# victorca25/iNNfer

Measured on AMD Instinct MI355X. Metric: output MPix/s, 4x ESRGAN RRDB-23 1080p->4K, higher is better.
Workload: dtype f16; 1 GPU; ESRGAN RRDBNet-23 4x fp16, 1x3x1080x1920 -> 1x3x4320x7680, un-tiled (Model(chop=False)), one frame per rank; band_rows=0, parallelism=single GPU

## Files before the change

include/innfer_amd.h:

```cpp
#ifndef INNFER_AMD_H
#define INNFER_AMD_H

#include <stddef.h>
#include <stdint.h>

#ifdef __cplusplus
extern "C" {
#endif

typedef enum {
    INNFER_OK = 0,
    INNFER_ERR_INVALID = -1,
    INNFER_ERR_HIP = -2,
    INNFER_ERR_UNSUPPORTED = -3,
    INNFER_ERR_NOMEM = -4,
    INNFER_ERR_WORKSPACE = -5
} innfer_status;

typedef enum { INNFER_F16 = 0, INNFER_F32 = 1, INNFER_U8 = 2  } innfer_dtype;

typedef struct innfer_net* innfer_net_t;

#define INNFER_ABI_VERSION 122
int innfer_version(void);
const char* innfer_last_error(void);


int innfer_rrdbnet_create(innfer_net_t* out, int in_nc, int out_nc, int nf, int nb,
                          int gc, int scale, int plus);

int innfer_rrdbnet_create_ex(innfer_net_t* out, int in_nc, int out_nc, int nf, int nb,
                             int gc, int scale, int plus, int nr, int act, int pixelshuffle_up);

int innfer_rrdbnet_create_ex2(innfer_net_t* out, int in_nc, int out_nc, int nf, int nb,
                              int gc, int scale, int plus, int nr, int act, int pixelshuffle_up, int unshuffle);
int innfer_first_conv_unshuffle(const void* d_in, int in_dtype, int normalize, int fp16_mode, int N, int in_nc, int H, int W, int unshuffle,
                                const float* h_weight_oihw, const float* h_bias, int K, int act, void* d_slab, int64_t group_stride, int64_t lo, void* stream);

int innfer_srresnet_create(innfer_net_t* out, int in_nc, int out_nc, int nf, int nb, int scale);
int innfer_srresnet_create_ex(innfer_net_t* out, int in_nc, int out_nc, int nf, int nb, int scale, int act, float res_scale, int upconv_up);
int innfer_net_set_conv_input_map(innfer_net_t net, int idx, const float* h_alpha, const float* h_shift, int act);

int innfer_compact_create(innfer_net_t* out, int in_nc, int out_nc, int nf, int num_conv, int scale);
int innfer_net_set_conv_slope(innfer_net_t net, int idx, const float* h_slope);

int innfer_net_set_precision(innfer_net_t net, int fp32);

void innfer_net_destroy(innfer_net_t net);

int innfer_net_num_convs(innfer_net_t net);
int innfer_net_conv_info(innfer_net_t net, int idx, char* key, size_t key_cap, int* K, int* C);

int innfer_net_set_conv(innfer_net_t net, int idx, const float* h_weight_oihw, const float* h_bias);

int innfer_net_scale(innfer_net_t net);
size_t innfer_net_workspace_bytes(innfer_net_t net, int N, int H, int W);

int innfer_net_forward(innfer_net_t net, const void* d_in, int in_dtype, void* d_out, int out_dtype,
                       int N, int H, int W, void* d_workspace, size_t workspace_bytes, void* stream);

int innfer_net_forward_timed(innfer_net_t net, const void* d_in, int in_dtype, void* d_out, int out_dtype,
                             int N, int H, int W, void* d_workspace, size_t workspace_bytes, void* stream,
                             int cap, float* h_ms, double* h_flops, double* h_bytes, int* h_kind, int* n_launches);

int innfer_net_set_u8_io(innfer_net_t net, int normalize, int fp16_mode);

int innfer_net_set_band_rows(innfer_net_t net, int rows);

int innfer_net_set_residual_lds(innfer_net_t net, int on);

int innfer_net_set_fused_tail(innfer_net_t net, int on);
int innfer_net_set_hr_chain(innfer_net_t net, int on);

int innfer_net_set_upconv_phases(innfer_net_t net, int mode);

int innfer_net_set_final_act(innfer_net_t net, int act);

int innfer_net_set_outm(innfer_net_t net, int outm);

double innfer_net_flops(innfer_net_t net, int N, int H, int W);

typedef struct innfer_unet* innfer_unet_t;
int innfer_unet_create(innfer_unet_t* out, int in_nc, int out_nc, int num_downs, int ngf);
int innfer_unet_create_ex(innfer_unet_t* out, int in_nc, int out_nc, int num_downs, int ngf, int instance_norm, int upconv);
void innfer_unet_destroy(innfer_unet_t u);
int innfer_unet_num_params(innfer_unet_t u);
int innfer_unet_param_info(innfer_unet_t u, int idx, char* key, size_t key_cap, int* ndim, int* shape4);
int innfer_unet_set_param(innfer_unet_t u, int idx, const float* h_data);
int innfer_unet_set_eval(innfer_unet_t u, int eval_mode);
int innfer_unet_set_precision(innfer_unet_t u, int fp32);
size_t innfer_unet_workspace_bytes(innfer_unet_t u, int N, int H, int W);
double innfer_unet_flops(innfer_unet_t u, int N, int H, int W);
int innfer_unet_forward(innfer_unet_t u, const void* d_in, int in_dtype, void* d_out, int out_dtype,
                        int N, int H, int W, void* d_workspace, size_t workspace_bytes, void* stream);

typedef struct innfer_pan* innfer_pan_t;
int innfer_pan_create(innfer_pan_t* out, int in_nc, int out_nc, int nf, int unf, int nb, int scale);
int innfer_pan_create_ex(innfer_pan_t* out, int in_nc, int out_nc, int nf, int unf, int nb, int scale, int self_attention, int double_scpa, int bilinear_up);
void innfer_pan_destroy(innfer_pan_t p);
int innfer_pan_num_params(innfer_pan_t p);
int innfer_pan_param_info(innfer_pan_t p, int idx, char* key, size_t key_cap, int* ndim, int* shape4);
int innfer_pan_set_param(innfer_pan_t p, int idx, const float* h_data);
size_t innfer_pan_workspace_bytes(innfer_pan_t p, int N, int H, int W);
int innfer_pan_set_fused_scpa(innfer_pan_t p, int on);
int innfer_pan_set_precision(innfer_pan_t p, int fp32);
int innfer_pan_forward(innfer_pan_t p, const void* d_in, int in_dtype, void* d_out, int out_dtype,
                       int N, int H, int W, void* d_workspace, size_t workspace_bytes, void* stream);

typedef struct innfer_ppon* innfer_ppon_t;
int innfer_ppon_create(innfer_ppon_t* out, int in_nc, int out_nc, int nf, int nb, int scale, float alpha);
void innfer_ppon_destroy(innfer_ppon_t p);
int innfer_ppon_num_params(innfer_ppon_t p);
int innfer_ppon_param_info(innfer_ppon_t p, int idx, char* key, size_t key_cap, int* ndim, int* shape4);
int innfer_ppon_set_param(innfer_ppon_t p, int idx, const float* h_data);
size_t innfer_ppon_workspace_bytes(innfer_ppon_t p, int N, int H, int W);
int innfer_ppon_set_precision(innfer_ppon_t p, int fp32);
int innfer_ppon_forward(innfer_ppon_t p, const void* d_in, int in_dtype, void* d_out_c, void* d_out_s, void* d_out_p,
                        int out_dtype, int N, int H, int W, void* d_workspace, size_t workspace_bytes, void* stream);

typedef struct innfer_resnet* innfer_resnet_t;
int innfer_resnet_create(innfer_resnet_t* out, int in_nc, int out_nc, int ngf, int n_blocks);
int innfer_resnet_create_ex(innfer_resnet_t* out, int in_nc, int out_nc, int ngf, int n_blocks, int padding, int use_dropout, int upconv, int batch_norm);
// ... 32 lines not shown
    const void* d_packed; const float* d_bias;
    void* d_out; int64_t out_group_stride; int out_ch_off; int K;
    int N, H, W;
    int act; int upsample2x;
    const void* d_res1; int64_t res1_group_stride; float res1_scale;
    const void* d_res2; int64_t res2_group_stride; float res2_scale;
    int row_begin, row_end;
    int reflect_pad;
    int dilation;
    int dilation_groups;
    int pixel_shuffle2;
    int stride2_k4;
    int transposed2x;
    int column7;
    int split;
    int64_t in_lo, out_lo, res1_lo, res2_lo;
    int reserved0;
    int res1_from_input;
    int plane_rows;
    float* d_stats_part;
    int64_t stats_part_floats;
    int conv1x1;
    int prefix_lrelu;
    const void* d_gate_packed;
    const float* d_gate_bias;
    int in_relu;
    int conv7x7;
    int out_planar;
    int out_denorm, out_round16;
    int planar_phases;
    int outm;
} innfer_conv_args;

size_t innfer_conv3x3_packed_bytes(int K, int C);
int innfer_pack_conv3x3(const float* h_weight_oihw, int K, int C, void* h_packed);
int innfer_pack_conv3x3_rows(const float* h_weight_oihw, int K, int C, int plane_rows, void* h_packed);
int innfer_pack_convt2x_rows(const float* h_weight_iohw, int K, int C, int k, int plane_rows, void* h_packed);
int innfer_pack_conv3x3_shuffle2(const float* h_weight_oihw, const float* h_bias, int K, int C, void* h_packed, float* h_bias_out);
size_t innfer_conv7x1_packed_bytes(int K, int C);
int innfer_pack_conv7x1(const float* h_weight_oc7, int K, int C, void* h_packed);
size_t innfer_conv4x4s2_packed_bytes(int K, int C);
int innfer_pack_conv4x4s2(const float* h_weight_oihw, int K, int C, void* h_packed);
size_t innfer_convt2x_packed_bytes(int K, int C);
int innfer_pack_convt2x(const float* h_weight_iohw, int K, int C, int k, void* h_packed);
size_t innfer_conv1x1_packed_bytes(int K, int C);
int innfer_pack_conv1x1(const float* h_weight_oi, int K, int C, void* h_packed);
int innfer_pack_conv1x1_split(const float* h_weight_oi, int K, int C, void* h_packed);
int innfer_pack_selfgate(const float* h_weight_32x32, void* h_packed_2k);
size_t innfer_conv7x7_packed_bytes(int K, int C);
int innfer_pack_conv7x7(const float* h_weight_oihw, int K, int C, void* h_packed);
int innfer_pack_up2x_phases(const float* h_weight_oihw, int K, int C, int plane_rows, void* h_packed);
int innfer_conv3x3_f16(const innfer_conv_args* a, void* stream);
int innfer_conv3x3_f16_slope(const innfer_conv_args* a, const float* d_slope, void* stream);
int innfer_shuffle_add(const void* d_slab, int64_t group_stride, const void* d_base, int base_dtype, int normalize, void* d_out, int out_dtype,
                       int N, int C, int H, int W, int scale, void* stream);
int innfer_pack_conv3x3_split(const float* h_weight_oihw, int K, int C, void* h_packed);

typedef struct {
    const float* d_in; int64_t in_nstride, in_cstride; int C, Hin, Win;
    const float* d_packed; const float* d_bias; int K;
    float* d_out; int64_t out_nstride, out_cstride, out_pstride; int Wout;
    int Ho, Wo;
    int osy, osx, ooy, oox;
    int isy, isx;
    int ntap, dy[49], dx[49];
    int pad_mode;
    int up;
    int in_act;
    int act;
    float oscale;
    const float* d_res; int64_t res_nstride, res_cstride;
    const float* d_mul; int64_t mul_nstride, mul_cstride;
    int N;
    int phase_k;
    int form;
} innfer_f32conv_args;

size_t innfer_f32conv_packed_floats(int K, int C, int ntap);
int innfer_pack_f32conv(const float* h_w, int K, int C, int ntap, float* h_packed);
int innfer_f32conv(const innfer_f32conv_args* a, void* stream);
int innfer_f32conv_plan(const innfer_f32conv_args* a, int* plan);
int innfer_f32_norm(const float* d_in, int64_t in_ns, int64_t in_cs, float* d_out, int64_t out_ns, int64_t out_cs, int N, int C, int64_t HW, int mode, float eps,
                    const float* d_weight, const float* d_bias, const float* d_rmean, const float* d_rvar, int act,
                    const float* d_res, int64_t res_ns, int64_t res_cs, int form, void* stream);

int innfer_conv_stats_records(int H, int W, int phases);
int innfer_norm_combine_parts(const float* d_part, int nper, int64_t HW, float eps, const float* d_gamma, const float* d_beta, float* d_alpha, float* d_shift,
                              int C, int N, void* stream);
int innfer_norm_stats(const void* d_src, int slab, int64_t gs, int cpad, int64_t HW, float eps, const float* d_gamma, const float* d_beta, float* d_alpha, float* d_shift,
                      int C, int N, float* d_part, int64_t part_floats, void* stream);
int innfer_resnet_post_slab_parts(const void* d_src, int64_t gs, int C, int64_t HW, int N, const float* d_part, int nper, const float* d_gamma, const float* d_beta,
                                  int relu, const void* d_res, void* d_dst, void* stream);
int innfer_unet_post_slab_parts(const void* d_src, int64_t src_gs, int C, int64_t HW, int N, const float* d_part, int nper, const float* d_gamma, const float* d_beta,
                                void* d_dst0, int64_t dst0_gs, int dst0_coff, int act0, void* d_dst1, int64_t dst1_gs, int dst1_coff, int act1, void* stream);

typedef struct {
    const void* d_in; int64_t in_group_stride; int cin_pad;
    const void* d_packed; int cout_pad;
    float* d_raw; int raw_stride, cout_store;
    int N, Hin, Win, Ho, Wo, stride;
    int ntaps, dy[49], dx[49];
    int Hfull, Wfull, os, ooy, oox, up, reflect;
    int ngroup; int64_t g_wbytes, g_outoff; int g_tapmul, g_phase;
    float* d_scratch; int64_t scratch_bytes;
    int keep_partials;
} innfer_gather_gemm_args;
// ... 124 lines not shown
```

innfer_amd/architectures/engine_module.py:

```python
import ctypes as C

import numpy as np
import torch
from torch import nn

from .. import lib as L


class _Node(nn.Module):
    """Anonymous container used to spell dotted key paths ("model.1.sub.0...")."""


def _result_tensor(out, shape, x):
    if out is None:
        return torch.empty(shape, dtype=x.dtype, device=x.device)
    if tuple(out.shape) != tuple(shape) or out.dtype != x.dtype or out.device != x.device or not out.is_contiguous():
        raise ValueError(f'out= must be a contiguous {tuple(shape)} {x.dtype} tensor on {x.device}; got {tuple(out.shape)} {out.dtype} on {out.device}'
                         f'{"" if out.is_contiguous() else ", not contiguous"}')
    return out


class EngineModule(nn.Module):
    def __init__(self, shapes):
        super().__init__()
        for key, shape in shapes.items():
            *path, leaf = key.split('.')
            node = self
            for name in path:
                if name not in node._modules:
                    node.add_module(name, _Node())
                node = node._modules[name]
            if leaf == 'num_batches_tracked':
                node.register_buffer(leaf, torch.zeros(shape, dtype=torch.long))
            elif leaf.startswith('running_'):
                node.register_buffer(leaf, torch.ones(shape) if leaf == 'running_var' else torch.zeros(shape))
            else:
                node.register_parameter(leaf, nn.Parameter(torch.zeros(*shape), requires_grad=False))
        self._handle = None
        self._uploaded_version = None
        self._weights_device = None
        self._ws = None
        self.band_rows = 0
        self.upconv_phases = True
        self.hr_chain = True
        self.fused_tail = True
        self.residual_lds = 1

    unshuffle = 1

    def _io_sizes(self, H, W, s):
        r = self.unshuffle
        return (-(-H // r) * s, -(-W // r) * s), (H * s // r, W * s // r)

    def _create_handle(self):
        raise NotImplementedError

    def _param_key(self, engine_key):
        return engine_key

    def _weights_version(self):
        ts = self.__dict__.get('_version_tensors')
        if ts is None:
            ts = list(self.parameters()) + list(self.buffers())
            self.__dict__['_version_tensors'] = ts
        return tuple([(t.data_ptr(), t._version) for t in ts])

    def invalidate_weights(self):
        self.__dict__.pop('_version_tensors', None)

    def _apply(self, fn, *args, **kwargs):
        r = super()._apply(fn, *args, **kwargs)
        self.invalidate_weights()
        return r

    def load_state_dict(self, *args, **kwargs):
        r = super().load_state_dict(*args, **kwargs)
        self.invalidate_weights()
        return r

    def _ensure_engine(self):
        ver = self._weights_version()
        if self._handle is not None and ver == self._uploaded_version:
            return
        if self._handle is None:
            self._handle = self._create_handle()
        sd = self.state_dict()
        n = L.lib.innfer_net_num_convs(self._handle)
        key = C.create_string_buffer(128)
        K, Cc = C.c_int(), C.c_int()
        for i in range(n):
            L.check(L.lib.innfer_net_conv_info(self._handle, i, key, 128, C.byref(K), C.byref(Cc)))
            k = self._param_key(key.value.decode())
            w, b = self._conv_tensors(k, sd)
            w = np.ascontiguousarray(w)
            if w.shape[:2] != (K.value, Cc.value):
                raise RuntimeError(f'size mismatch for {k}.weight: {tuple(w.shape)} vs engine ({K.value},{Cc.value},3,3)')
            bp = None
            if b is not None:
# ... 16 lines not shown
                pass
        self._handle, self._uploaded_version, self._ws = None, None, None

    def __del__(self):
        try:
            self._destroy_handle()
        except Exception:
            pass

    _OUTM = {None: 0, 'scaltanh': 1, 'tanh': 2, 'sigmoid': 3, 'clamp': 4}

    _accepts_out = True

    def forward(self, x, outm=None, out=None):
        self._outm = self._OUTM.get(outm, 0)
        if not isinstance(x, torch.Tensor) or x.dim() != 4:
            raise ValueError('expected a 4D [N,C,H,W] tensor')
        if not x.is_cuda:
            raise RuntimeError(
                'innfer_amd runs its forward on an MI355X only: there is no CPU path '
                '(the CPU restatement lives in oracle/ and is test infrastructure).')
        if x.dtype not in (torch.float16, torch.float32):
            raise TypeError(f'unsupported dtype {x.dtype}')
        with torch.cuda.device(x.device):
            return self._forward_on_device(x, out)

    def _engine_on(self, device):
        device = torch.device(device)
        if device.index is None:
            device = torch.device('cuda', torch.cuda.current_device())
        if self._weights_device is not None and self._weights_device != device:
            self._destroy_handle()
        self._ensure_engine()
        self._weights_device = device

    def _home_device(self, device=None):
        if device is not None:
            device = torch.device(device)
            return device if device.index is not None else torch.device('cuda', torch.cuda.current_device())
        if self._weights_device is not None:
            return self._weights_device
        for p in self.parameters():
            if p.is_cuda:
                return p.device
            break
        return torch.device('cuda', torch.cuda.current_device())

    def _forward_on_device(self, x, out=None):
        self._engine_on(x.device)
        L.check(L.lib.innfer_net_set_band_rows(self._handle, int(self.band_rows)))
        L.check(L.lib.innfer_net_set_fused_tail(self._handle, int(bool(self.fused_tail))))
        L.check(L.lib.innfer_net_set_hr_chain(self._handle, int(bool(self.hr_chain))))
        L.check(L.lib.innfer_net_set_residual_lds(self._handle, int(self.residual_lds)))
        L.check(L.lib.innfer_net_set_upconv_phases(self._handle, int(self.upconv_phases)))
        L.check(L.lib.innfer_net_set_outm(self._handle, int(getattr(self, '_outm', 0))))
        L.check(L.lib.innfer_net_set_precision(self._handle, int(x.dtype == torch.float32)))
        x = x.contiguous()
        N, _, H, W = x.shape
        s = L.lib.innfer_net_scale(self._handle)
        full, want = self._io_sizes(H, W, s)
        out = _result_tensor(out, (N, self.out_nc) + want, x)
        res = out if full == want else torch.empty((N, self.out_nc) + full, dtype=x.dtype, device=x.device)
        need = L.lib.innfer_net_workspace_bytes(self._handle, N, H, W)
        if self._ws is None or self._ws.numel() < need or self._ws.device != x.device:
            self._ws = None
            self._ws = torch.empty(need, dtype=torch.uint8, device=x.device)
        dt = L.F16 if x.dtype == torch.float16 else L.F32
        stream = torch.cuda.current_stream(x.device).cuda_stream
        L.check(L.lib.innfer_net_forward(self._handle, x.data_ptr(), dt, res.data_ptr(), dt, N, H, W,
                                         self._ws.data_ptr(), self._ws.numel(), stream))
        if res is not out:
            out.copy_(res[:, :, :want[0], :want[1]])
        return out

    def forward_u8(self, img, normalize=False, fp16=True, out=None):
        if not isinstance(img, torch.Tensor) or img.dtype != torch.uint8 or img.dim() not in (3, 4):
            raise ValueError('forward_u8: expected a uint8 [H,W,C] or [N,H,W,C] tensor')
        if not img.is_cuda:
            raise RuntimeError('innfer_amd runs its forward on an MI355X only: there is no CPU path')
        with torch.cuda.device(img.device):
            self._engine_on(img.device)
            L.check(L.lib.innfer_net_set_band_rows(self._handle, int(self.band_rows)))
            L.check(L.lib.innfer_net_set_fused_tail(self._handle, int(bool(self.fused_tail))))
            L.check(L.lib.innfer_net_set_hr_chain(self._handle, int(bool(self.hr_chain))))
            L.check(L.lib.innfer_net_set_residual_lds(self._handle, int(self.residual_lds)))
            L.check(L.lib.innfer_net_set_upconv_phases(self._handle, int(self.upconv_phases)))
            L.check(L.lib.innfer_net_set_u8_io(self._handle, int(bool(normalize)), int(bool(fp16))))
            L.check(L.lib.innfer_net_set_precision(self._handle, int(not fp16)))
            L.check(L.lib.innfer_net_set_outm(self._handle, 0))
            x = img.contiguous()
            batched = x.dim() == 4
            N, (H, W, Cc) = (x.shape[0] if batched else 1), x.shape[-3:]
            if Cc != self.in_nc:
                raise ValueError(f'forward_u8: the image has {Cc} channels, the network takes {self.in_nc}')
            s = L.lib.innfer_net_scale(self._handle)
            full, want = self._io_sizes(H, W, s)
            shape = (N,) + want + (self.out_nc,) if batched else want + (self.out_nc,)
            if out is None:
                out = torch.empty(shape, dtype=torch.uint8, device=x.device)
            elif tuple(out.shape) != shape or out.dtype != torch.uint8 or not out.is_contiguous():
                raise ValueError(f'forward_u8: out must be a contiguous uint8 tensor of shape {shape}')
            need = L.lib.innfer_net_workspace_bytes(self._handle, N, H, W)
            if self._ws is None or self._ws.numel() < need or self._ws.device != x.device:
                self._ws = None
                self._ws = torch.empty(need, dtype=torch.uint8, device=x.device)
            res = out if full == want else torch.empty((N,) + full + (self.out_nc,), dtype=torch.uint8, device=x.device)
            L.check(L.lib.innfer_net_forward(self._handle, x.data_ptr(), L.U8, res.data_ptr(), L.U8, N, H, W,
                                             self._ws.data_ptr(), self._ws.numel(), torch.cuda.current_stream(x.device).cuda_stream))
            if res is not out:
                out.copy_(res[:, :want[0], :want[1]] if batched else res[0, :want[0], :want[1]])
        return out

    def release_workspace(self):
        self._ws = None

    def tile_batch_bytes(self, b, ps, dtype=torch.float16, device=None):
        device = self._home_device(device)
        with torch.cuda.device(device):
            self._engine_on(device)
            L.check(L.lib.innfer_net_set_precision(self._handle, int(dtype == torch.float32)))
            elt = 4 if dtype == torch.float32 else 2
            s = L.lib.innfer_net_scale(self._handle)
            (hh, ww), _ = self._io_sizes(ps, ps, s)
            return L.lib.innfer_net_workspace_bytes(self._handle, b, ps, ps) + b * (self.in_nc * ps * ps + 2 * self.out_nc * hh * ww) * elt

    def _out_shape(self, N, H, W, device=None):
        device = self._home_device(device)
        with torch.cuda.device(device):
            self._engine_on(device)
            s = L.lib.innfer_net_scale(self._handle)
        return (N, self.out_nc) + self._io_sizes(H, W, s)[1]

    def flops(self, N, H, W, device=None):
        device = self._home_device(device)
        with torch.cuda.device(device):
            self._engine_on(device)
            return L.lib.innfer_net_flops(self._handle, N, H, W)
```

innfer_amd/csrc/common.h:

```cpp
#pragma once
#include <hip/hip_runtime.h>
#include <atomic>
#include <cstdarg>
#include <cstdint>
#include <cstdio>
#include <cstdlib>
#include <functional>
#include <string>
#include <vector>

#include "../../include/innfer_amd.h"

namespace innfer {

typedef _Float16 f16;
typedef _Float16 f16x8 __attribute__((ext_vector_type(8)));
typedef _Float16 f16x4 __attribute__((ext_vector_type(4)));
typedef float f32x4 __attribute__((ext_vector_type(4)));
typedef unsigned u32x4 __attribute__((ext_vector_type(4)));

int set_error(int code, const char* fmt, ...);

__device__ __forceinline__ float fast_sigmoid(float x) { return __builtin_amdgcn_rcpf(1.0f + __expf(-x)); }
__device__ __forceinline__ float fast_tanh(float x) { return 1.0f - 2.0f * __builtin_amdgcn_rcpf(1.0f + __expf(2.0f * x)); }
// ... 31 lines not shown
    if (!(done.load(std::memory_order_acquire) & bit)) {
        const hipError_t e = hipFuncSetAttribute((const void*)kernel, hipFuncAttributeMaxDynamicSharedMemorySize, lds_bytes);
        if (e != hipSuccess) return e;
        done.fetch_or(bit, std::memory_order_release);
    }
    return hipSuccess;
}

struct XcdRun { int start, len, slots, j0; };
__device__ __forceinline__ XcdRun xcd_run(int total) {
    const int bid = blockIdx.x, xcd = bid & 7;
    const int q = total >> 3, r = total & 7;
    return {xcd < r ? xcd * (q + 1) : r * (q + 1) + (xcd - r) * q, q + (xcd < r ? 1 : 0), ((int)gridDim.x + 7 - xcd) >> 3, bid >> 3};
}

enum OutMode { OUT_SLAB = 0, OUT_NCHW = 1, OUT_SHUFFLE2 = 2 };
#include "conv3x3_modes.h"

struct ConvLaunch {
    const f16* in; long in_gstride; int C;
    const f16* wpk; const float* bias;
    void* out; long out_gstride;
    int out_coff;
    int K;
    int N, H, W;
    int act; int up;
    const f16* res1; long res1_gstride; float s1;
    const f16* res2; long res2_gstride; float s2;
    int y0, y1;
    int out_mode; int out_f32;
    int rev;
    int deconv_phases;
    int stride2;
    float* stats_part;
    int prefix_lrelu;
    int conv1x1;
    int dilation_groups;
    int dilation;
    int conv7v;
    int conv7;
    int reflect;
    const f16* fuse_w;
    const float* fuse_bias; float* fuse_side; void* fuse_out; int fuse_oc, fuse_out_mode;
    int phase_c;
    int outm;
    int out_u8, out_denorm, out_round16;
    int split;
    long in_lo, out_lo, res1_lo, res2_lo;
    int rowp;
    int in_relu;
    const f16* gate_w; const float* gate_bias;
    const float* slope;
    int res1_lds;
};

int conv_nt_for(int K);
size_t conv_packed_bytes(int K, int C);
void conv_pack_shuffle2(const float* w_oihw, const float* bias, int K, int C, void* packed, float* bias_out);
void conv_pack(const float* w_oihw, int K, int C, void* packed, int rowp = 0);
void conv_pack_split(const float* w_oihw, int K, int C, void* packed);
void conv_pack_1x1_split(const float* w_oi, int K, int C, void* packed);
int conv_launch(const ConvLaunch& L, hipStream_t s);
size_t conv_packed_bytes_taps(int K, int C, int mask);
void conv_pack_selfgate(const float* w32x32, void* packed_2k);
void conv_pack_1x1(const float* w_oi, int K, int C, void* packed);
int conv_stats_nper(int H, int W, int phases);
size_t conv_packed_bytes7v(int K, int C);
void conv_pack7v(const float* w_oc7, int K, int C, void* packed);
size_t conv_packed_bytes_s2k4(int K, int C);
void conv_pack_s2k4(const float* w_oi44, int K, int C, void* packed);
size_t conv_packed_bytes_deconv2x(int K, int C);
bool conv_fuse_last_ok(const ConvLaunch& L);
size_t conv_fuse_side_bytes(int N, int H, int W);
void conv_pack_fuse_last(const float* w_last_oihw, int oc, void* packed_4k, int rowp = 0, int cin = 64);
void conv_pack_up2x_phases(const float* w_oihw, int K, int C, void* packed, int rowp = 0);
void conv_pack_deconv2x(const float* w_io, int K, int C, int k, void* packed, int rowp = 0);
void conv_pack_taps(const float* w, int K, int C, int mask, void* packed, int rowp = 0);
size_t conv_packed_bytes7x7(int K, int C);
void conv_pack7x7(const float* w_oihw, int K, int C, void* packed);

bool hr_chain_ok(const ConvLaunch& L);
int hr_chain_launch(const ConvLaunch& L, const f16* up_in, long up_in_gstride, const f16* up_wpk, const float* up_bias, int up_act, hipStream_t s);

struct FirstConvLaunch {
    const void* in; int in_f32; int Cin;
    int in_u8, in_norm, in_round16;
    const float* w;
    const float* bias;
    f16* out; long out_gstride; f16* out2; long out2_gstride;
    int K; int N, H, W; int act;
    long out_lo, out2_lo;
    const float* slope;
};
int first_conv_launch(const FirstConvLaunch& L, hipStream_t s);

struct FirstUnshuffleLaunch {
    const void* in; int in_f32; int Cin;
    int in_u8, in_norm, in_round16;
    int r;
    const void* wpk;
    const float* bias;
    f16* out; long out_gstride; f16* out2; long out2_gstride;
    int K; int N, H, W; int act;
    long out_lo, out2_lo;
};
size_t first_unshuffle_packed_bytes(int K, int r);
// ... 61 lines not shown
```

innfer_amd/csrc/conv3x3.hip:

```cpp
#include "common.h"
#include <type_traits>

#include <cstdlib>
#include <cstring>
#include <vector>

#define FP32_VALUE(x) asm("" : "+v"(x))
#ifndef INNFER_IN_AUX
#define INNFER_IN_AUX 0
#endif

#pragma clang fp contract(off)

namespace innfer {

#ifdef INNFER_STAMPS
#define NSTAMP 16
__device__ unsigned long long g_stamps[8192 * NSTAMP];
#define STAMP(i)                                                                              \
    do {                                                                                      \
        if (blockIdx.x < 8192 && threadIdx.x == 0)                                            \
            g_stamps[blockIdx.x * NSTAMP + (i)] = (unsigned long long)clock64();              \
    } while (0)
#else
// ... 311 lines not shown
                    for (int t = 0; t < 4; ++t) h[t] = (f16)v[t][j];
                    *(f16x4*)op = h;
                } else {
#pragma unroll
                    for (int t = 0; t < NT; ++t) op[t] = (f16)v[t][j];
                }
            }
        }
    }
#ifdef INNFER_STAMPS
    STAMP(13);
    asm volatile("s_waitcnt vmcnt(0)" ::: "memory");
    STAMP(12);
    if (blockIdx.x < 8192 && threadIdx.x == 0) g_stamps[blockIdx.x * NSTAMP + 15] = (unsigned long long)wall_clock64();
#endif
    }
}


#ifdef INNFER_STAMPS
#define PCT(var) const unsigned long long var = clock64()
#define PCACC(slot, t1, t0) do { if (lane == 0 && blockIdx.x < 8192) g_stamps[blockIdx.x * NSTAMP + (slot)] += (t1) - (t0); } while (0)
#else
#define PCT(var) do { } while (0)
#define PCACC(slot, t1, t0) do { } while (0)
#endif
#include "conv3x3_fuse.h"

#include "conv3x3_stats_gate_rlds.h"

#include "conv3x3_planar.h"

__device__ __forceinline__ f16x8 relu_frag(f16x8 b) {
    typedef unsigned u32x4_t __attribute__((ext_vector_type(4)));
    u32x4_t v = __builtin_bit_cast(u32x4_t, b);
#pragma unroll
    for (int e = 0; e < 4; ++e) { unsigned o; asm("v_pk_max_f16 %0, %1, 0" : "=v"(o) : "v"(v[e])); v[e] = o; }
    return __builtin_bit_cast(f16x8, v);
}

template <int RPW, int NT, int NLW, int OUTMODE, bool S9 = false, bool POLY = false, int TMF = TAPS_3X3, bool CV = false, int NSI = 2, int NCW = 8>
__global__ __launch_bounds__(64 * (NCW + NLW), 1) void conv3x3_pc(const KP p) {
    constexpr int TM = TMF & TAPS_3X3;
    constexpr bool S2 = (TMF & PC_S2) != 0;
    constexpr bool PAIR = (TMF & PC_PAIR) != 0;
    constexpr int NSEG = 2;
    constexpr int TWI = PAIR ? 16 : TW;
    static_assert(!PAIR || (__builtin_popcount(TM) == 4 && !S9 && !POLY && !CV), "image pairs: the four-tap kernels");
    constexpr bool PFX = (TMF & PC_PFX) != 0;
    constexpr bool STATS = (TMF & PC_STATS) != 0;
    constexpr bool SPLIT = (TMF & PC_SPLIT) != 0;
    static_assert(!SPLIT || (!S9 && !POLY && !S2 && !PFX && !STATS && (TM == TAPS_3X3 || TM == TAPS_1X1)), "split operands: plain 3x3 and 1x1 convs");
    constexpr bool RLDS = (TMF & PC_RLDS) != 0;
    static_assert(!RLDS || (RPW == 2 && NT == 4 && NCW == 8 && NSI == 2 && OUTMODE == OUT_SLAB && (TMF & PC_BELOW_RLDS) == TAPS_3X3 && !S9 && !POLY), "residual from LDS: the plain 64-channel instantiation (and its canvas form)");
    constexpr bool SGATE = (TMF & PC_SGATE) != 0;
    static_assert(!SGATE || (RPW == 3 && NT == 2 && NCW == 8 && OUTMODE == OUT_SLAB && ((TMF & PC_BELOW_SGATE) == TAPS_3X3 || (TMF & PC_BELOW_SGATE) == (TAPS_3X3 | PC_SPLIT)) && !S9 && !POLY), "self gate: the 32-output slab kernel (its canvas form, its split-operand form)");
    constexpr bool BRELU = (TMF & PC_BRELU) != 0;
    constexpr bool UP4 = (TMF & PC_UP4) != 0;
    constexpr bool ROWP = (TMF & PC_ROWP) != 0;
    static_assert(!ROWP || (RPW == 2 && NT == 4 && NCW == 8 && OUTMODE == OUT_SLAB && TM == TAPS_3X3 && (TMF & ~(TAPS_3X3 | PC_FUSE | PC_RLDS | PC_UP4 | PC_ROWP | PC_PSH | PC_PRELU)) == 0 && !S9 && !POLY), "plane row order: the 64-channel slab kernels");
    constexpr bool PSH = (TMF & PC_PSH) != 0;
    static_assert(!PSH || (ROWP && (TMF & ~(TAPS_3X3 | PC_ROWP | PC_PSH)) == 0 && NSI == 2 && !CV), "pixel-shuffle store: the plain 64-channel plane-order instantiation");
    static_assert(!UP4 || (RPW == 2 && NT == 4 && NCW == 8 && NSI == 3 && OUTMODE == OUT_SLAB && (TMF & PC_BELOW_UP4) == TAPS_3X3 && !S9 && !POLY && !CV), "one-pass phases: the 64-channel slab kernel on three input slots");
    constexpr bool FUSE = (TMF & PC_FUSE) != 0;
    constexpr bool PRELU = (TMF & PC_PRELU) != 0;
    static_assert(!PRELU || (OUTMODE == OUT_SLAB && (NT == 4 || NT == 2) && NCW == 8 && NSI == 2 && (TMF & ~(TAPS_3X3 | PC_ROWP | PC_PRELU)) == 0 && TM == TAPS_3X3 && !S9 && !POLY && !CV), "PReLU epilogue: the plain 64- / 32-output slab kernels");
    static_assert(!FUSE || (RPW == 2 && (NT == 4 || (NT == 2 && !ROWP)) && NCW == 8 && NSI == 2 && OUTMODE == OUT_SLAB && (TMF & PC_BELOW_FUSE) == TAPS_3X3 && !S9 && !POLY && !CV), "the fused last conv: the plain 64-channel instantiation (and the 32-channel one on 16-row tiles)");
    using L = PcLayout<RPW, NT, NSI, NCW, TMF>;
    constexpr int TH = L::TH;
    constexpr int LH = TH + 2;
    constexpr int NPX = LH * LWP;
    constexpr int IN_BYTES = L::IN_BYTES;
    constexpr int NQ = IN_BYTES / 1024;
    constexpr int KQ = (NQ + NLW - 1) / NLW;
    constexpr int WROWS = NT * 16;
    constexpr int NTAP = L::NTAP;
    constexpr int W_BYTES = L::W_BYTES;
    constexpr int WQ = W_BYTES / 1024;
    constexpr int KW = (WQ + NLW - 1) / NLW;
    constexpr int MT = RPW * 2;
    constexpr int STAGE = L::STAGE;
    constexpr int OOB = (int)0x80000000;
#ifdef INNFER_NO_PIPE
    constexpr bool PIPE = false;
#else
    constexpr bool PIPE = true;
#endif
#ifdef INNFER_NO_PIPE4
    constexpr bool PIPE4 = false;
#else
    constexpr bool PIPE4 = true;
#endif

    extern __shared__ __attribute__((aligned(16))) char smem[];
    const int tid = threadIdx.x;
    const int lane = tid & 63;
    const int wave = __builtin_amdgcn_readfirstlane(tid >> 6);
    const int li = lane & 15, lg = lane >> 4;

    const XcdRun run = xcd_run(p.total);
    const int run_start = run.start, run_len = run.len, slots = run.slots, j0 = run.j0;
    const int per_img = p.tiles_x * p.tiles_y;
    if (j0 >= run_len) return;
    const int ntiles = (run_len - j0 + slots - 1) / slots;
    const int G = ntiles * p.nchunks;

    auto decode = [&](int jj, int& kg_, int& n_, int& ty0_, int& tx0_) __attribute__((always_inline)) {
        const int lid = run_start + (p.rev ? run_len - 1 - jj : jj);
        kg_ = lid % p.KG;
        int tile = lid / p.KG;
        n_ = tile / per_img;
        tile -= n_ * per_img;
        const int ty = tile / p.tiles_x;
        ty0_ = p.y0 + ty * TH;
        tx0_ = (tile - ty * p.tiles_x) * TW;
        if constexpr (TM == TAPS_PHASE) {
            const int ph = kg_ * WROWS / p.phase_c;
            ty0_ += ph >> 1; tx0_ += ph & 1;
        }
    };
    auto decode_poly = [&](int jj, int& kg_, int& n_, int& ty0_, int& tx0_, int& d_) {
        if (p.nrate == 0) { decode(jj, kg_, n_, ty0_, tx0_); d_ = p.dil; return; }
        const int lid = run_start + (p.rev ? run_len - 1 - jj : jj);
        int r = 0;
        while (r + 1 < p.nrate && lid >= p.rate_start[r + 1]) ++r;
        kg_ = r; d_ = r + 1;
        int tile = lid - p.rate_start[r];
        const int tx = ((p.fullW + d_ - 1) / d_ + TW - 1) / TW, ty = ((p.fullH + d_ - 1) / d_ + TH - 1) / TH;
        n_ = tile / (tx * ty);
        tile -= n_ * tx * ty;
        const int row = tile / tx;
        ty0_ = row * TH;
        tx0_ = (tile - row * tx) * TW;
    };

#include "conv3x3_pc_loaders.inc"

#if defined(INNFER_CPRIO) && defined(__HIP_DEVICE_COMPILE__)
    __builtin_amdgcn_s_setprio(INNFER_CPRIO);
#endif
    const int cw = wave;
    int boffs[3][2];
#pragma unroll
    for (int s = 0; s < 3; ++s)
#pragma unroll
        for (int par = 0; par < 2; ++par) {
            const int pb = cw * RPW * LWP + li + s;
            const int rowpar = ((cw * RPW) & 1) ^ par;
            boffs[s][par] = pb * 64 + ((lg ^ (((((li + s) >> 2) & 1) ^ rowpar) << 1)) << 4);
        }
    int boffp[PAIR ? 3 : 1][2];
    if constexpr (PAIR) {
#pragma unroll
        for (int s = 0; s < 3; ++s)
#pragma unroll
            for (int par = 0; par < 2; ++par) {
                const int pb = cw * RPW * LWP + 18 + li + s;
                const int rowpar = ((cw * RPW) & 1) ^ par;
                boffp[s][par] = pb * 64 + ((lg ^ (((((18 + li + s) >> 2) & 1) ^ rowpar) << 1)) << 4);
            }
    }
    const int aoffs = li * 64 + ((lg ^ (((li >> 2) & 1) << 1)) << 4);
    int roffs[RLDS ? MT : 1];
    if constexpr (RLDS) {
#pragma unroll
        for (int m = 0; m < MT; ++m) {
            const int P = (cw * RPW + (m >> 1) + 1) * LWP + li + (m & 1) * 16 + 1;
            roffs[m] = P * 64 + (((lg & 1) ^ ((P >> 2) & 1)) << 5);
            if constexpr (ROWP) roffs[m] = P * 64 + ((lg ^ (((P >> 2) & 1) << 1)) << 4);
        }
    }
    f16x8 sgw[SGATE ? 2 : 1];
    [[maybe_unused]] f16x8 sgwl[(SGATE && SPLIT) ? 2 : 1];
    f32x4 sgb[SGATE ? 2 : 1];
    if constexpr (SGATE) {
#pragma unroll
        for (int t = 0; t < 2; ++t) {
            sgw[t] = *(const f16x8*)(p.sg_w + (t * 64 + lane) * 8);
            if constexpr (SPLIT) sgwl[t] = *(const f16x8*)(p.sg_w + 1024 + (t * 64 + lane) * 8);
            sgb[t] = *(const f32x4*)(p.sg_bias + 8 * lg + 4 * t);
        }
    }
    auto four_tap = [&](auto tmc, f32x4 (&acc)[NT][2 * RPW], const char* st, const char* sw) __attribute__((always_inline)) {
        constexpr int TMX = decltype(tmc)::value;
        constexpr const TapWalk& WK = TapWalkOf<TMX, RPW, NSEG>::value;
        constexpr int NBW = TapWalkOf<TMX, RPW, NSEG>::value.n;
        constexpr int R0 = (TMX & 0x007) ? 0 : 1, S0 = (TMX & 0x049) ? 0 : 1;
        static_assert(TMX == (TAPS_PHASE << (3 * R0 + S0)), "four taps: a 2 x 2 block of the 3 x 3 lattice");
        f16x8 a[2][NT];
        auto lda = [&](int sc, int q) {
#pragma unroll
            for (int t = 0; t < NT; ++t) a[q][t] = *(const f16x8*)(sw + aoffs + ((q * 2 + sc - S0) * WROWS + t * 16) * 64);
        };
        f16x8 bq[3];
        auto ldb = [&](int i) {
            if constexpr (PAIR) { if (WK.seg[i]) return *(const f16x8*)(st + boffp[WK.s[i]][WK.rr[i] & 1] + WK.rr[i] * LWP * 64); }
            return *(const f16x8*)(st + boffs[WK.s[i]][WK.rr[i] & 1] + (WK.rr[i] * LWP + WK.seg[i] * 16) * 64);
        };
        lda(S0, 0); lda(S0, 1);
        bq[0] = ldb(0);
        if (NBW > 1) bq[1] = ldb(1);
        if constexpr (BRELU) bq[0] = relu_frag(bq[0]);
#pragma unroll
        for (int i = 0; i < NBW; ++i) {
            if (i + 2 < NBW) bq[(i + 2) % 3] = ldb(i + 2);
#pragma unroll
            for (int q = 0; q < 2; ++q) {
                const int rw = WK.rr[i] - R0 - q;
                if (rw >= 0 && rw < RPW) {
#pragma unroll
                    for (int t = 0; t < NT; ++t)
                        acc[t][rw * 2 + WK.seg[i]] = __builtin_amdgcn_mfma_f32_16x16x32_f16(a[q][t], bq[i % 3], acc[t][rw * 2 + WK.seg[i]], 0, 0, 0);
                }
            }
            if constexpr (BRELU) { if (i + 1 < NBW) bq[(i + 1) % 3] = relu_frag(bq[(i + 1) % 3]); }
            if (WK.s[i] == S0 && WK.seg[i] == NSEG - 1) {
                if (WK.rr[i] == R0 + RPW - 1) lda(S0 + 1, 0);
                if (WK.rr[i] == R0 + RPW) lda(S0 + 1, 1);
            }
            __builtin_amdgcn_sched_barrier(0);
        }
    };
#include "conv3x3_pc_up4.inc"
    int islot = 0;
    f32x4 bias_r[NT];
    [[maybe_unused]] float* slope_lds = (float*)(smem + L::TAIL) + cw * 64;
    if constexpr (PRELU) { if (lane < WROWS) slope_lds[lane] = p.slope[lane]; }
    int bias_kg = -1;
    f32x4 acc[NT][MT];
    float pfx[PFX ? MT : 1][8];
#pragma unroll
    for (int m = 0; m < (PFX ? MT : 1); ++m)
#pragma unroll
        for (int e = 0; e < 8; ++e) pfx[m][e] = 0.f;
    int jt = j0, c = 0;
    int kg = 0, n = 0, ty0 = 0, tx0 = 0, cbase = 0, dcur = 1;
    asm volatile("s_barrier" ::: "memory");
#ifdef INNFER_STAMPS
    const unsigned long long k_c0 = clock64(), k_w0 = wall_clock64();
#endif
    for (int g = 0; g < G; ++g) {
        if (c == 0) {
            if constexpr (POLY) decode_poly(jt, kg, n, ty0, tx0, dcur);
            else decode(jt, kg, n, ty0, tx0);
            cbase = kg * WROWS + lane_cbase<NT, ROWP>(lg);
            if (kg != bias_kg) {
#pragma unroll
                for (int t = 0; t < NT; ++t) bias_r[t] = *(const f32x4*)(p.bias + cbase + toff_lin<NT, ROWP>(t));
                bias_kg = kg;
            }
#pragma unroll
            for (int t = 0; t < NT; ++t)
#pragma unroll
                for (int m = 0; m < MT; ++m) acc[t][m] = SPLIT ? f32x4{0.f, 0.f, 0.f, 0.f} : bias_r[t];
        }
        if constexpr (SPLIT) {
            if (c == 2 * p.ncg) {
#pragma unroll
                for (int t = 0; t < NT; ++t)
#pragma unroll
                    for (int m = 0; m < MT; ++m)
#pragma unroll
                        for (int j = 0; j < 4; ++j) acc[t][m][j] = __builtin_fmaf(acc[t][m][j], SPLIT_DOWN, bias_r[t][j]);
            }
        }
        const char* st = NSI == 3 ? smem + islot * IN_BYTES : smem + (g & 1) * STAGE;
        const char* sw = NSI == 3 ? smem + 3 * IN_BYTES + (g & 1) * W_BYTES : st + IN_BYTES;
        if constexpr (NSI == 3) islot = islot == 2 ? 0 : islot + 1;
        PCT(c0);
#ifdef INNFER_ABLATE
        const bool abl_no_mfma = (p.abl & 8) != 0;
#else
        constexpr bool abl_no_mfma = false;
#endif
        if (abl_no_mfma) {
        } else if constexpr (TM == TAPS_3X3 && PIPE && !UP4) {
            constexpr int GPS = 2 * (RPW + 2);
            constexpr int NB = 3 * GPS;
            f16x8 a[3][NT];
            f16x8 bq[3];
            auto lda = [&](int sc, int r) {
#pragma unroll
                for (int t = 0; t < NT; ++t) a[r][t] = *(const f16x8*)(sw + aoffs + ((r * 3 + sc) * WROWS + t * 16) * 64);
            };
            auto ldb = [&](int i) {
                const int sc = i / GPS, j = i - sc * GPS, rr = j >> 1, seg = j & 1;
                return *(const f16x8*)(st + boffs[sc][rr & 1] + (rr * LWP + seg * 16) * 64);
            };
            lda(0, 0); lda(0, 1); lda(0, 2);
            bq[0] = ldb(0); bq[1] = ldb(1);
            if constexpr (BRELU) bq[0] = relu_frag(bq[0]);
#pragma unroll
            for (int i = 0; i < NB; ++i) {
                const int sc = i / GPS, j = i - sc * GPS, rr = j >> 1, seg = j & 1;
                if (i + 2 < NB) bq[(i + 2) % 3] = ldb(i + 2);
#pragma unroll
                for (int r = 0; r < 3; ++r) {
                    const int rw = rr - r;
                    if (rw >= 0 && rw < RPW) {
#pragma unroll
                        for (int t = 0; t < NT; ++t)
                            acc[t][rw * 2 + seg] = __builtin_amdgcn_mfma_f32_16x16x32_f16(a[r][t], bq[i % 3], acc[t][rw * 2 + seg], 0, 0, 0);
                    }
                }
                if constexpr (BRELU) { if (i + 1 < NB) bq[(i + 1) % 3] = relu_frag(bq[(i + 1) % 3]); }
                if (sc < 2 && seg == 1) {
                    if (rr == RPW - 1) lda(sc + 1, 0);
                    if (rr == RPW) lda(sc + 1, 1);
                    if (rr == RPW + 1) lda(sc + 1, 2);
                }
                __builtin_amdgcn_sched_barrier(0);
            }
        } else if constexpr (NTAP == 4 && !PFX && PIPE4 && RPW <= 6 && !UP4) {
            four_tap(std::integral_constant<int, TM>{}, acc, st, sw);
        } else {
#pragma unroll
        for (int s = 0; s < 3; ++s) {
            if (!((TM >> s) & 0x49)) continue;
            f16x8 a[3][NT];
#pragma unroll
            for (int r = 0; r < 3; ++r)
#pragma unroll
                for (int t = 0; t < NT; ++t)
                    if ((TM >> (r * 3 + s)) & 1)
                        a[r][t] = *(const f16x8*)(sw + aoffs + (__builtin_popcount(TM & ((1 << (r * 3 + s)) - 1)) * WROWS + t * 16) * 64);
#pragma unroll
            for (int rr = 0; rr < RPW + 2; ++rr) {
                bool need = false;
#pragma unroll
                for (int r = 0; r < 3; ++r) need = need || (((TM >> (r * 3 + s)) & 1) && rr - r >= 0 && rr - r < RPW);
                if (!need) continue;
#pragma unroll
                for (int seg = 0; seg < NSEG; ++seg) {
                    f16x8 b = *(const f16x8*)(st + ((PAIR && seg) ? boffp[PAIR ? s : 0][rr & 1] + rr * LWP * 64 : boffs[s][rr & 1] + (rr * LWP + seg * 16) * 64));
                    if constexpr (BRELU) b = relu_frag(b);
                    if constexpr (PFX) {
                        static_assert(!PFX || TM == TAPS_1X1, "the running-sum operand belongs to the one-tap kernels");
#pragma unroll
                        for (int e = 0; e < 8; ++e) {
                            float& run = pfx[PFX ? (rr - 1) * 2 + seg : 0][e];
                            run += (float)b[e];
                            b[e] = (f16)fmaxf(run, 0.2f * run);
                        }
                    }
#pragma unroll
                    for (int r = 0; r < 3; ++r) {
                        const int rw = rr - r;
                        if (((TM >> (r * 3 + s)) & 1) && rw >= 0 && rw < RPW) {
#pragma unroll
                            for (int t = 0; t < NT; ++t)
                                acc[t][rw * 2 + seg] = __builtin_amdgcn_mfma_f32_16x16x32_f16(
                                    a[r][t], b, acc[t][rw * 2 + seg], 0, 0, 0);
                        }
                    }
                }
            }
        }
        }
        if constexpr (RLDS) {
            if constexpr (ROWP) {
                if (c == p.nchunks - 2) residual_from_lds_plane<MT, 0>(acc, st, roffs, p.rs1);
                else if (c == p.nchunks - 1) residual_from_lds_plane<MT, 1>(acc, st, roffs, p.rs1);
            } else {
                if (c >= p.nchunks - 2 && (lg >> 1) == c - (p.nchunks - 2)) residual_from_lds<MT>(acc, st, roffs, p.rs1);
            }
        }
        PCT(c1);
        if (cw == 0) PCACC(0, c1, c0);
        if (++c == p.nchunks) {
            c = 0;
            jt += slots;
            if constexpr (SGATE && SPLIT) self_gate_split<MT>(acc, sgw, sgwl, sgb);
            else if constexpr (SGATE) self_gate<MT>(acc, sgw, sgb);
            if constexpr (PFX) {
#pragma unroll
                for (int m = 0; m < MT; ++m)
#pragma unroll
                    for (int e = 0; e < 8; ++e) pfx[m][e] = 0.f;
            }
#include "conv3x3_pc_tile_end.inc"
        }
        PCT(c2);
#ifdef INNFER_ABLATE
        if ((p.abl & 32) && c != 0) continue;
#endif
        asm volatile("s_barrier" ::: "memory");
        PCT(c3);
        if (cw == 0) { PCACC(1, c2, c1); PCACC(2, c3, c2); PCACC(6, 1, 0); }
    }
#ifdef INNFER_STAMPS
    if (cw == 0) { PCACC(7, clock64(), k_c0); PCACC(8, wall_clock64(), k_w0); }
#endif
}

template <int RPW, int NT, int NLW, int OUTMODE = OUT_SLAB, bool S9 = false, bool POLY = false, int TM = TAPS_3X3, bool CV = false, int NSI = 2, int NCW = 8>
int launch_pc(const KP& kp, int N, hipStream_t s);

int num_cus() {
    static int n[64] = {};
    const int dev = current_device() & 63;
    if (!n[dev]) {
        int v = 0;
        if (hipDeviceGetAttribute(&v, hipDeviceAttributeMultiprocessorCount, dev) != hipSuccess || v <= 0) v = 256;
        n[dev] = v;
    }
    return n[dev];
}

template <int RPW, int NT, int OUTMODE>
int launch_t(const KP& kp, int N, hipStream_t s) {
    constexpr int TH = 4 * RPW;
    constexpr int LDS = (((TH + 2) * LWP + 15) / 16) * 1024 + 9 * NT * 16 * 64 + ((RPW == 3 && NT == 2) ? 0 : 2048);
    static std::atomic<unsigned long long> attr_done{0};
    INNFER_HIP(ensure_lds_attr(conv3x3_mfma<RPW, NT, OUTMODE>, LDS, attr_done));
    KP k = kp;
    k.tiles_x = (k.W + TW - 1) / TW;
    k.tiles_y = (k.y1 - k.y0 + TH - 1) / TH;
    {
        const int pf = INNFER_KNOB("INNFER_PREFETCH", 0);
        k.pf = (RPW == 3 && NT == 2) ? 0 : pf;
#ifdef INNFER_ABLATE
        k.abl = getenv("INNFER_ABL") ? atoi(getenv("INNFER_ABL")) : 0;
#endif
    }
    const long total = (long)N * k.tiles_x * k.tiles_y * k.KG;
    if (total <= 0) return INNFER_OK;
    if (total > 0x7fffffffL) return set_error(INNFER_ERR_INVALID, "conv grid too large");
    k.total = (int)total;
    const int persist = INNFER_KNOB("INNFER_PERSIST", 2);
    const long slots = (long)((persist == 2 && RPW == 3 && NT == 2) ? 3 : persist) * num_cus();
    const long grid = (persist > 0 && total > slots) ? slots : total;
    hipLaunchKernelGGL((conv3x3_mfma<RPW, NT, OUTMODE>), dim3((unsigned)grid), dim3(256), LDS, s, k);
    INNFER_HIP(hipGetLastError());
    return INNFER_OK;
}

template <int TH>
int canvas_grid(const KP& k, int N, int* gy, long* tiles) {
    const long plain = (long)N * ((k.W + TW - 1) / TW) * ((k.H + TH - 1) / TH);
    *tiles = plain; *gy = 0;
    if (N < 2 || k.up || k.reflect || (k.act >= 3 && k.act != 7) || k.y0 != 0 || k.y1 != k.H || k.H < TH + 2 || k.W < LVALID || k.nrate || k.dil > 1 || k.stats_part ||
        (long)N * k.H * k.W * 64 >= 0x7fffffffL)
        return 0;
    int best = 0;
    for (int gx = 1; gx <= N; ++gx) {
        const int g_y = (N + gx - 1) / gx;
        const long t = (long)((gx * (k.W + 1) + TW - 1) / TW) * ((g_y * (k.H + 1) + TH - 1) / TH);
        if (t < *tiles) { *tiles = t; best = gx; *gy = g_y; }
    }
    return *tiles * 100 <= plain * 98 ? best : 0;
}

template <int RPW, int NT, int NLW, int OUTMODE, bool S9, bool POLY, int TM, bool CV, int NSI, int NCW>
int launch_pc(const KP& kp, int N, hipStream_t s) {
    constexpr int TH = NCW * RPW;
    constexpr int LDS = PcLayout<RPW, NT, NSI, NCW, TM>::LDS_BYTES;
    static_assert(LDS <= 160 * 1024, "the stages must fit the CU's LDS");
    static_assert(NSI == 2 || (NSI == 3 && !S9 && !POLY), "the three-slot input ring exists for the plain and the canvas loader");
    if constexpr (OUTMODE == OUT_SLAB && !S9 && !POLY && (TM & ~(PC_SPLIT | PC_RLDS | PC_SGATE | PC_ROWP)) == TAPS_3X3 && !CV) {
        int gy = 0; long t = 0;
        const int gx = INNFER_KNOB("INNFER_CANVAS", 1) ? canvas_grid<TH>(kp, N, &gy, &t) : 0;
        if (gx > 0) {
            KP kc = kp;
            kc.cv_gx = gx; kc.cv_gy = gy; kc.cv_h1 = kp.H + 1; kc.cv_w1 = kp.W + 1;
            return launch_pc<RPW, NT, NLW, OUTMODE, false, false, TM, true, NSI, NCW>(kc, N, s);
        }
    }
    static std::atomic<unsigned long long> attr_done{0};
    INNFER_HIP(ensure_lds_attr(conv3x3_pc<RPW, NT, NLW, OUTMODE, S9, POLY, TM, CV, NSI, NCW>, LDS, attr_done));
    KP k = kp;
    k.tiles_x = (k.W + TW - 1) / TW;
    k.tiles_y = (k.y1 - k.y0 + TH - 1) / TH;
    k.N = N;
#ifdef INNFER_ABLATE
    k.abl = getenv("INNFER_ABL") ? atoi(getenv("INNFER_ABL")) : 0;
#endif
    long total = (long)((TM & PC_PAIR) ? (N + 1) / 2 : N) * k.tiles_x * k.tiles_y * k.KG;
    if constexpr (CV) {
        k.tiles_x = (k.cv_gx * k.cv_w1 + TW - 1) / TW;
        k.tiles_y = (k.cv_gy * k.cv_h1 + TH - 1) / TH;
        total = (long)k.tiles_x * k.tiles_y * k.KG;
    }
    if (POLY && k.nrate > 0) {
        total = 0;
        for (int g = 0; g < k.nrate; ++g) {
            const int d = g + 1;
            k.rate_start[g] = (int)total;
            total += (long)N * d * d * (((k.fullW + d - 1) / d + TW - 1) / TW) * (((k.fullH + d - 1) / d + TH - 1) / TH);
        }
        if (total <= 0x7fffffffL) k.rate_start[k.nrate] = (int)total;
    }
    if (total <= 0) return INNFER_OK;
    if (total > 0x7fffffffL) return set_error(INNFER_ERR_INVALID, "conv grid too large");
    k.total = (int)total;
    const long grid = total < num_cus() ? total : num_cus();
    hipLaunchKernelGGL((conv3x3_pc<RPW, NT, NLW, OUTMODE, S9, POLY, TM, CV, NSI, NCW>), dim3((unsigned)grid), dim3(64 * (NCW + NLW)), LDS, s, k);
    INNFER_HIP(hipGetLastError());
    return INNFER_OK;
}

}

}
#ifdef INNFER_STAMPS
namespace innfer { __global__ void k_clear_stamps() { for (int i = threadIdx.x; i < 8192 * NSTAMP; i += blockDim.x) g_stamps[i] = 0; } }
#endif
extern "C" int innfer_debug_clear_stamps() {
#ifdef INNFER_STAMPS
// ... 167 lines not shown
        k.nchunks = 4 * k.ncg;
        if (nt == 2) return launch_pc<3, 2, 4, OUT_SLAB, false, false, TAPS_S2 | PC_S2>(k, L.N, s);
        if (L.stats_part) return L.W <= 16 ? launch_pc<2, 4, 4, OUT_SLAB, false, false, TAPS_S2 | PC_S2 | PC_PAIR | PC_STATS, false, UNET_NSI>(k, L.N, s) : launch_pc<2, 4, 4, OUT_SLAB, false, false, TAPS_S2 | PC_S2 | PC_STATS, false, UNET_NSI>(k, L.N, s);
        return L.W <= 16 ? launch_pc<2, 4, 4, OUT_SLAB, false, false, TAPS_S2 | PC_S2 | PC_PAIR, false, UNET_NSI>(k, L.N, s) : launch_pc<2, 4, 4, OUT_SLAB, false, false, TAPS_S2 | PC_S2, false, UNET_NSI>(k, L.N, s);
    }
    if (L.conv7v) {
        if (!pc || L.out_mode != OUT_SLAB || (nt != 2 && nt != 4) || L.res1 || L.res2 || L.up || L.act > 2 || L.y0 != 0 || k.y1 != L.H || L.reflect == 2 ||
            (long)L.H * L.W * 64 >= 0x7fffffffL)
            return set_error(INNFER_ERR_UNSUPPORTED, "conv7x1: slab output of 32- / 64-channel tiles, no residual / upsampling, images below 33 M pixels");
        k.nchunks = 3 * k.ncg; k.s9v = 1;
        if (L.stats_part) return launch_pc<2, 4, 4, OUT_SLAB, true, false, TAPS_COL | PC_STATS>(k, L.N, s);
        return nt == 4 ? launch_pc<2, 4, 4, OUT_SLAB, true, false, TAPS_COL>(k, L.N, s) : launch_pc<3, 2, 4, OUT_SLAB, true, false, TAPS_COL>(k, L.N, s);
    }
    if (L.conv1x1) {
        if (!pc || L.out_mode != OUT_SLAB || (nt != 2 && nt != 4))
            return set_error(INNFER_ERR_UNSUPPORTED, "conv1x1: slab outputs of 32- / 64-channel tiles on the producer-consumer kernel");
        if (L.prefix_lrelu) {
            if (nt != 4) return set_error(INNFER_ERR_UNSUPPORTED, "conv1x1: the running-sum operand is built for 64-channel tiles");
            return launch_pc<2, 4, 4, OUT_SLAB, false, false, TAPS_1X1 | PC_PFX>(k, L.N, s);
        }
        return nt == 4 ? launch_pc<2, 4, 4, OUT_SLAB, false, false, TAPS_1X1, false, 3>(k, L.N, s) : launch_pc<2, 2, 4, OUT_SLAB, false, false, TAPS_1X1, false, 3>(k, L.N, s);
    }
    if (L.gate_w) {
        if (!pc || L.out_mode != OUT_SLAB || nt != 2 || L.K != 32 || L.res1 || L.res2 || L.act > 2 || L.reflect || L.stats_part)
            return set_error(INNFER_ERR_UNSUPPORTED, "conv3x3: the self gate belongs to 32-output slab convs without residuals (act = the activation AFTER the gate)");
        k.sg_w = L.gate_w; k.sg_bias = L.gate_bias;
        return launch_pc<3, 2, 4, OUT_SLAB, false, false, TAPS_3X3 | PC_SGATE>(k, L.N, s);
    }
    if (pc && L.out_mode == OUT_SLAB && nt == 2 && !L.fuse_w) {
        if (pc == 5) return launch_pc<2, 2, 4, OUT_SLAB, false, false, TAPS_3X3, false, 3>(k, L.N, s);
        if (INNFER_KNOB("INNFER_FAT", 0) & 1) return launch_pc<6, 2, 4, OUT_SLAB, false, false, TAPS_3X3, false, 2, 4>(k, L.N, s);
        return pc == 2 ? launch_pc<3, 2, 8>(k, L.N, s) : pc == 3 ? launch_pc<2, 2, 4>(k, L.N, s) : launch_pc<3, 2, 4>(k, L.N, s);
    }
    if (L.fuse_w) {
        if (!conv_fuse_last_ok(L)) return set_error(INNFER_ERR_UNSUPPORTED, "conv3x3: the fused last conv needs 64 or 32 output channels, whole 16 x 32 tiles, act 0..2, no residual / upsampling / row range");
        k.fl_w = L.fuse_w; k.fl_bias = L.fuse_bias; k.fl_side = L.fuse_side; k.fl_out = L.fuse_out; k.fl_oc = L.fuse_oc; k.fl_out_mode = L.fuse_out_mode;
        if (nt == 2 && L.rowp) return set_error(INNFER_ERR_UNSUPPORTED, "conv3x3: the fused last conv behind a 32-channel conv takes lane-contiguous panels");
        if (int rc = nt == 2 ? launch_pc<2, 2, 4, OUT_SLAB, false, false, TAPS_3X3 | PC_FUSE>(k, L.N, s)
                             : L.rowp ? launch_pc<2, 4, 4, OUT_SLAB, false, false, TAPS_3X3 | PC_FUSE | PC_ROWP>(k, L.N, s) : launch_pc<2, 4, 4, OUT_SLAB, false, false, TAPS_3X3 | PC_FUSE>(k, L.N, s)) return rc;
        const long nthr = (long)L.N * (L.H / 16) * (L.W / 32) * 92;
        hipLaunchKernelGGL(fuse_combine_kernel, dim3((unsigned)((nthr + 255) / 256)), dim3(256), 0, s, (const float*)L.fuse_side, L.fuse_bias, L.fuse_out, L.fuse_out_mode, L.out_denorm, L.out_round16, L.fuse_oc,
                           L.N, L.H, L.W);
        INNFER_HIP(hipGetLastError());
        return INNFER_OK;
    }
    if (L.out_mode == OUT_SHUFFLE2 && L.rowp == 2) {
        if (!pc || nt != 4 || L.K % 256 || L.res1 || L.res2 || L.up || L.reflect || L.act > 2 || L.y0 != 0 || k.y1 != L.H || L.stats_part ||
            (long)L.N * L.H * L.W * 64 * 4 >= 0x7fffffffL)
            return set_error(INNFER_ERR_UNSUPPORTED, "conv3x3: the phase-major PixelShuffle(2) store needs K %% 256 == 0 (64-channel phases), act 0..2, no residual / upsampling / row range, < 2 GiB per output group");
        k.phase_c = L.K / 4;
        return launch_pc<2, 4, 4, OUT_SLAB, false, false, TAPS_3X3 | PC_ROWP | PC_PSH>(k, L.N, s);
    }
    if (pc && L.out_mode == OUT_SLAB && nt == 4 && L.stats_part) return launch_pc<2, 4, 4, OUT_SLAB, false, false, TAPS_3X3 | PC_STATS>(k, L.N, s);
    if (pc && L.out_mode == OUT_SLAB && nt == 4 && L.res1_lds && L.res1 && L.res1 == L.in && L.res1_gstride == L.in_gstride && L.act == 0 && L.K == 64 && L.C >= 96 &&
        !L.up && !L.reflect && L.s1 != 0.f && (L.res1_lds == 2 || L.res2)) {
        k.rs1 = 1.0f / L.s1;
        return L.rowp ? launch_pc<2, 4, 4, OUT_SLAB, false, false, TAPS_3X3 | PC_RLDS | PC_ROWP>(k, L.N, s) : launch_pc<2, 4, 4, OUT_SLAB, false, false, TAPS_3X3 | PC_RLDS>(k, L.N, s);
    }
    if (pc && L.out_mode == OUT_SLAB && nt == 4) {
        if (!L.rowp && (INNFER_KNOB("INNFER_FAT", 0) & 2)) return launch_pc<4, 4, 4, OUT_SLAB, false, false, TAPS_3X3, false, 2, 4>(k, L.N, s);
        return L.rowp ? launch_pc<2, 4, 4, OUT_SLAB, false, false, TAPS_3X3 | PC_ROWP>(k, L.N, s) : launch_pc<2, 4, 4>(k, L.N, s);
    }
    if (L.conv7) {
        if (!pc || L.out_mode != OUT_NCHW || nt != 1 || L.res1 || L.res2 || L.up || (long)L.H * L.W * 64 >= 0x7fffffffL)
            return set_error(INNFER_ERR_UNSUPPORTED, "conv7x7: planar output with K <= 16, no residual / upsampling, images below 33 M pixels");
        k.nchunks = 9 * k.ncg;
        return launch_pc<3, 1, 4, OUT_NCHW, true>(k, L.N, s);
    }
    if (pc && L.out_mode == OUT_NCHW && nt == 1 && !L.res1 && !L.res2) return launch_pc<3, 1, 4, OUT_NCHW>(k, L.N, s);
    if (pc && L.out_mode == OUT_NCHW && nt == 2 && !L.res1 && !L.res2 && !L.phase_c && !L.reflect && !L.out_u8) return launch_pc<3, 2, 4, OUT_NCHW>(k, L.N, s);
    if (L.act >= 3 || L.phase_c > 0 || L.reflect)
        return set_error(INNFER_ERR_UNSUPPORTED, "conv3x3: tanh / phase output / gate epilogues / reflection padding exist only in the producer-consumer kernel");
    switch (L.out_mode) {
        case OUT_SLAB:
            if (nt == 4) return rpw64 == 4 ? launch_t<4, 4, OUT_SLAB>(k, L.N, s) : rpw64 == 3 ? launch_t<3, 4, OUT_SLAB>(k, L.N, s) : launch_t<2, 4, OUT_SLAB>(k, L.N, s);
            if (nt == 2) return rpw32 == 6 ? launch_t<6, 2, OUT_SLAB>(k, L.N, s) : rpw32 == 5 ? launch_t<5, 2, OUT_SLAB>(k, L.N, s) : rpw32 == 3 ? launch_t<3, 2, OUT_SLAB>(k, L.N, s) : launch_t<4, 2, OUT_SLAB>(k, L.N, s);
            return launch_t<4, 1, OUT_SLAB>(k, L.N, s);
        case OUT_NCHW:
            if (nt == 4) return launch_t<2, 4, OUT_NCHW>(k, L.N, s);
            if (nt == 2) return launch_t<4, 2, OUT_NCHW>(k, L.N, s);
            return launch_t<4, 1, OUT_NCHW>(k, L.N, s);
        case OUT_SHUFFLE2:
            if (nt == 4) return launch_t<2, 4, OUT_SHUFFLE2>(k, L.N, s);
            return set_error(INNFER_ERR_UNSUPPORTED, "pixelshuffle conv needs K %% 64 == 0");
    }
    return set_error(INNFER_ERR_INVALID, "conv3x3: bad out_mode");
}

}
```

innfer_amd/csrc/conv3x3_epilogue_slab.h:

```cpp

constexpr float ACT_TOP = 3.0e38f;

template <int NT, bool ROWP>
__device__ __forceinline__ long toff_slab(int t, long g) { return (NT == 4 && ROWP) ? (long)(t >> 1) * g + 4 * (t & 1) : 4 * t; }
template <int NT, bool ROWP>
__device__ __forceinline__ int toff_lin(int t) { return (NT == 4 && ROWP) ? 32 * (t >> 1) + 4 * (t & 1) : 4 * t; }
template <int NT, bool ROWP>
__device__ __forceinline__ int lane_cbase(int lg) { return ((NT == 4 && ROWP) ? 8 : 4 * NT) * lg; }

template <int RPW, int NT, int ACT, bool R1, bool R2, bool SC1 = false, bool ROWP = false>
__device__ __forceinline__ void epilogue_slab_cv(const KP& p, f32x4 (&acc)[NT][2 * RPW], int ty0, int tx0, int wave, int li, int cbase) {
    constexpr int MT = 2 * RPW;
    constexpr int NTS = ACT == 7 ? NT / 2 : NT;
    const int oc0 = (ACT == 7 ? cbase >> 1 : cbase) + p.out_coff;
    const int cyB = ty0 / p.cv_h1, yB = ty0 - cyB * p.cv_h1 + wave * RPW;
    const int cxB = tx0 / p.cv_w1, xB = tx0 - cxB * p.cv_w1 + li;
    f16* ob = (f16*)p.out + (oc0 >> 5) * p.out_gstride + (oc0 & 31);
    const f16* r1b = R1 ? p.res1 + (cbase >> 5) * p.res1_gstride + (cbase & 31) : nullptr;
    const f16* r2b = R2 ? p.res2 + (cbase >> 5) * p.res2_gstride + (cbase & 31) : nullptr;
    bool ok[MT];
    int off[MT];
    f16x4 r1[R1 ? MT : 1][NT], r2[R2 ? MT : 1][NT];
#pragma unroll
    for (int m = 0; m < MT; ++m) {
// ... 42 lines not shown
            *(f16x4*)(op + toff_slab<NT, ROWP>(t, p.out_gstride)) = h;
        }
    }
}

template <int RPW, int NT, int ACT, bool R1, bool R2, bool HOIST, bool POLY = false, bool DCV = false, bool PAIR = false, bool SC1 = false, bool ROWP = false, bool PSH = false>
__device__ __forceinline__ void epilogue_slab(const KP& p, f32x4 (&acc)[NT][2 * RPW], int n, int ty0, int tx0,
                                              int wave, int li, int cbase, int dil = 1, const f32x4* slope = nullptr) {
    constexpr int MT = 2 * RPW;
    constexpr int NTS = ACT == 7 ? NT / 2 : NT;
    int oc0 = (ACT == 7 ? cbase >> 1 : cbase) + p.out_coff;
    int yw = ty0 + wave * RPW, xl = tx0 + li;
    long pix0 = ((long)n * p.H + yw) * p.W + xl;
#ifdef INNFER_ABLATE
    if (p.abl & 16) pix0 = (long)blockIdx.x * 64 + wave * RPW * p.W + li;
#endif
    long rowstep = (long)p.W * 32;
    long colstep = 16 * 32;
    int ylim = p.y1, xlim = p.W;
    if constexpr (POLY) {
        const int d = dil, dd = d * d;
        const int nn = n / dd, ph = n - nn * dd, py = ph / d, px = ph - py * d;
        pix0 = ((long)nn * p.fullH + (long)yw * d + py) * p.fullW + (long)xl * d + px;
        rowstep = (long)p.fullW * 32 * d;
        colstep = 16L * 32 * d;
        ylim = (p.fullH - py + d - 1) / d;
        xlim = (p.fullW - px + d - 1) / d;
    }
    if constexpr (DCV || PSH) {
        const int ph = cbase / p.phase_c, a = ph >> 1, b = ph & 1;
        oc0 -= ph * p.phase_c;
        if constexpr (!PSH) { yw -= a; xl -= b; }
        pix0 = ((long)n * 2 * p.H + 2 * yw + a) * (2 * p.W) + 2 * xl + b;
        rowstep = (long)p.W * 32 * 4;
        colstep = 16 * 32 * 2;
        ylim = p.H;
        if constexpr (PAIR) { pix0 = ((long)(2 * n) * 2 * p.H + 2 * yw + a) * (2 * p.W) + 2 * xl + b; colstep = 4L * p.H * p.W * 32; }
#ifdef INNFER_ABLATE
        if (!PAIR && (p.abl & 64)) { pix0 = ((long)n * 2 * p.H + 2 * yw + a) * (2 * p.W) + xl + b * p.W; colstep = 16 * 32; }
#endif
    } else if constexpr (PAIR) {
        pix0 = ((long)(2 * n) * p.H + yw) * p.W + xl;
        colstep = (long)p.H * p.W * 32;
    }
    f16* ob = (f16*)p.out + (oc0 >> 5) * p.out_gstride + pix0 * 32 + (oc0 & 31);
    const f16* r1b = R1 ? p.res1 + (cbase >> 5) * p.res1_gstride + pix0 * 32 + (cbase & 31) : nullptr;
    const f16* r2b = R2 ? p.res2 + (cbase >> 5) * p.res2_gstride + pix0 * 32 + (cbase & 31) : nullptr;
    bool ok[MT];
    f16x4 r1[R1 ? MT : 1][NT], r2[R2 ? MT : 1][NT];
#pragma unroll
    for (int m = 0; m < MT; ++m) {
        ok[m] = PAIR ? (2 * n + (m & 1) < p.N && yw + (m >> 1) < ylim && xl < xlim) : ((yw + (m >> 1) < ylim) && (xl + (m & 1) * 16 < xlim));
        const long o = (m >> 1) * rowstep + (m & 1) * colstep;
        if (HOIST && R1 && ok[m]) {
#pragma unroll
            for (int t = 0; t < NT; ++t) r1[R1 ? m : 0][t] = *(const f16x4*)(r1b + o + toff_slab<NT, ROWP>(t, p.res1_gstride));
        }
        if (HOIST && R2 && ok[m]) {
#pragma unroll
            for (int t = 0; t < NT; ++t) r2[R2 ? m : 0][t] = *(const f16x4*)(r2b + o + toff_slab<NT, ROWP>(t, p.res2_gstride));
        }
    }
#pragma unroll
    for (int m = 0; m < MT; ++m) {
        if (!ok[m]) continue;
#ifdef INNFER_ABLATE
        if (p.abl & 1) continue;
#endif
        f16* op = ob + (m >> 1) * rowstep + (m & 1) * colstep;
#ifdef INNFER_ABLATE
        if (DCV && !PAIR && (p.abl & 128)) op = (f16*)p.out + (pix0 - 2 * li) * 32 + (m * 64 + (int)(threadIdx.x & 63)) * 16;
        if (!DCV && !PAIR && !POLY && (p.abl & 256)) {
            const int lgq = (int)(threadIdx.x & 63) >> 4;
            if (NT == 2) op = op - li * 32 - 8 * lgq + (int)(threadIdx.x & 63) * 8;
            else if (NT == 4) op = op - li * 32 - 16 * (lgq & 1) + ((lgq & 1) * 16 + li) * 16;
        }
        if (!DCV && !PAIR && !POLY && (p.abl & 128)) op = (f16*)p.out + (pix0 - li) * 32 + (m * 64 + (int)(threadIdx.x & 63)) * (4 * NT);
#endif
        if (!HOIST) {
            const long o = (m >> 1) * rowstep + (m & 1) * colstep;
#pragma unroll
            for (int t = 0; t < NT; ++t) {
                if (R1) r1[R1 ? m : 0][t] = *(const f16x4*)(r1b + o + toff_slab<NT, ROWP>(t, p.res1_gstride));
                if (R2) r2[R2 ? m : 0][t] = *(const f16x4*)(r2b + o + toff_slab<NT, ROWP>(t, p.res2_gstride));
            }
        }
#pragma unroll
        for (int t = 0; t < NTS; ++t) {
            f16x4 h;
#pragma unroll
            for (int j = 0; j < 4; ++j) {
                float f = acc[t][m][j];
                if (ACT == 7) {
                    f = f * fast_sigmoid(acc[t + NT / 2][m][j]);
                } else if (ACT == 4 || ACT == 5) {
                    f = (float)r1[R1 ? m : 0][t][j] * (fast_sigmoid(f));
                    if (ACT == 4) f = fmaxf(f, 0.2f * f);
                } else {
                    if (ACT == 1) f = __builtin_amdgcn_fmed3f(f, 0.2f * f, ACT_TOP);
                    else if (ACT == 2) f = __builtin_amdgcn_fmed3f(f, 0.f, ACT_TOP);
                    else if (ACT == 8) f = f >= 0.f ? f : slope[t][j] * f;
                    if (SC1) { f = f * p.s1; FP32_VALUE(f); }
                    if (R1) f = __builtin_fmaf(f, p.s1, (float)r1[R1 ? m : 0][t][j]);
                    if (R2) f = __builtin_fmaf(f, p.s2, (float)r2[R2 ? m : 0][t][j]);
                }
                FP32_VALUE(f);
                h[j] = (f16)f;
            }
            *(f16x4*)(op + toff_slab<NT, ROWP>(t, p.out_gstride)) = h;
        }
    }
}

constexpr float SPLIT_UP = 2048.0f, SPLIT_DOWN = 1.0f / 2048.0f;
template <int RPW, int NT, int ACT, bool R1, bool R2, bool CV>
__device__ __forceinline__ void epilogue_slab_split(const KP& p, f32x4 (&acc)[NT][2 * RPW], int n, int ty0, int tx0, int wave, int li, int cbase) {
    constexpr int MT = 2 * RPW;
    const int oc0 = cbase + p.out_coff;
    f16* ob = (f16*)p.out + (oc0 >> 5) * p.out_gstride + (oc0 & 31);
    const f16* r1b = R1 ? p.res1 + (cbase >> 5) * p.res1_gstride + (cbase & 31) : nullptr;
    const f16* r2b = R2 ? p.res2 + (cbase >> 5) * p.res2_gstride + (cbase & 31) : nullptr;
    int cyB = 0, yB = 0, cxB = 0, xB = 0;
    if constexpr (CV) {
        cyB = ty0 / p.cv_h1; yB = ty0 - cyB * p.cv_h1 + wave * RPW;
        cxB = tx0 / p.cv_w1; xB = tx0 - cxB * p.cv_w1 + li;
    }
#pragma unroll
    for (int m = 0; m < MT; ++m) {
        bool ok;
        long off;
        if constexpr (CV) {
            int y = yB + (m >> 1), cy = cyB;
            if (y >= p.cv_h1) { y -= p.cv_h1; ++cy; }
            int x = xB + (m & 1) * 16, cx = cxB;
            if (x >= p.cv_w1) { x -= p.cv_w1; ++cx; }
            const int nn = cy * p.cv_gx + cx;
            ok = y < p.H && x < p.W && cy < p.cv_gy && cx < p.cv_gx && nn < p.N;
            off = (((long)nn * p.H + y) * p.W + x) * 32;
        } else {
            const int y = ty0 + wave * RPW + (m >> 1), x = tx0 + li + (m & 1) * 16;
            ok = y < p.y1 && x < p.W;
            off = (((long)n * p.H + y) * p.W + x) * 32;
        }
        if (!ok) continue;
        f16x4 r1h[NT], r1l[NT], r2h[NT], r2l[NT];
#pragma unroll
        for (int t = 0; t < NT; ++t) {
            if (R1) { r1h[t] = *(const f16x4*)(r1b + off + 4 * t); r1l[t] = *(const f16x4*)(r1b + p.res1_lo + off + 4 * t); }
            if (R2) { r2h[t] = *(const f16x4*)(r2b + off + 4 * t); r2l[t] = *(const f16x4*)(r2b + p.res2_lo + off + 4 * t); }
        }
#pragma unroll
        for (int t = 0; t < NT; ++t) {
            f16x4 h, l;
#pragma unroll
            for (int j = 0; j < 4; ++j) {
                float f = acc[t][m][j];
                if (ACT >= 4) {
                    f = __builtin_fmaf((float)r1l[t][j], SPLIT_DOWN, (float)r1h[t][j]) * fast_sigmoid(f);
                    if (ACT == 4) f = fmaxf(f, 0.2f * f);
                } else {
                    if (ACT == 1) f = __builtin_amdgcn_fmed3f(f, 0.2f * f, ACT_TOP);
                    else if (ACT == 2) f = __builtin_amdgcn_fmed3f(f, 0.f, ACT_TOP);
                    if (R1) f = __builtin_fmaf(f, p.s1, __builtin_fmaf((float)r1l[t][j], SPLIT_DOWN, (float)r1h[t][j]));
                    if (R2) f = __builtin_fmaf(f, p.s2, __builtin_fmaf((float)r2l[t][j], SPLIT_DOWN, (float)r2h[t][j]));
                }
                FP32_VALUE(f);
// ... 11 lines not shown
```

innfer_amd/csrc/conv3x3_kp.h:

```cpp
constexpr int TW = 32;
constexpr int LWP = 36;
constexpr int LVALID = TW + 2;

template <int RPW, int NT, int NSI, int NCW, int TMF>
struct PcLayout {
    static constexpr int TH = NCW * RPW;
    static constexpr int IN_BYTES = (((TH + 2) * LWP + 15) / 16) * 1024;
    static constexpr int NTAP = (TMF & PC_UP4) ? 4 : __builtin_popcount(TMF & TAPS_3X3);
    static constexpr int W_BYTES = NTAP * NT * 16 * 64;
    static constexpr int STAGE = IN_BYTES + W_BYTES;
    static constexpr int TAIL = NSI * IN_BYTES + 2 * W_BYTES;
    static constexpr int FUSE_BYTES = (TMF & PC_FUSE) ? 4096 : 0;
    static constexpr int UP4_BYTES = (TMF & PC_UP4) ? 1024 : 0;
    static constexpr int PRELU_BYTES = (TMF & PC_PRELU) ? NCW * 256 : 0;
    static_assert((FUSE_BYTES != 0) + (UP4_BYTES != 0) + (PRELU_BYTES != 0) <= 1, "the tail users share one offset: at most one per instantiation");
    static constexpr int LDS_BYTES = TAIL + FUSE_BYTES + UP4_BYTES + PRELU_BYTES;
};


struct KP {
    const f16* in; long in_img_stride; long in_gbytes; int nchunks;
    const f16* wpk; const float* bias;
    void* out; long out_gstride; int out_coff;
    int K, KG;
    int H, W, Hs, Ws;
    int act, up;
    const f16* res1; long res1_gstride; float s1;
    const f16* res2; long res2_gstride; float s2;
    int y0, y1;
    int tiles_x, tiles_y;
    int out_f32;
    int outm;
    int out_u8, out_denorm, out_round16;
    int N;
    int pf;
    int rev;
    int nrate, rate_start[9];
    int dil, fullH, fullW;
    int ncg;
    float* stats_part;
    int stats_cn;
    int s9v;
    int reflect;
    int phase_c;
    int total;
    int cv_gx, cv_gy, cv_h1, cv_w1;
    const f16* fl_w;
    const float* fl_bias;
    float* fl_side;
    void* fl_out;
    int fl_oc, fl_out_mode;
    const f16* sg_w;
    union {
        const float* sg_bias;
        const float* slope;
    };
    float rs1;
    long in_lo_bytes;
    long out_lo, res1_lo, res2_lo;
#ifdef INNFER_ABLATE
    int abl;
#endif
// ... 3 lines not shown
```

innfer_amd/csrc/conv3x3_modes.h:

```cpp

constexpr int TAPS_3X3   = 0x1FF;
constexpr int TAPS_1X1   = 0x010;
constexpr int TAPS_COL   = 0x092;
constexpr int TAPS_PHASE = 0x01B;
constexpr int TAPS_S2    = 0x1B0;

constexpr int PC_S2    = 0x200;
constexpr int PC_PAIR  = 0x400;
constexpr int PC_PFX   = 0x800;
constexpr int PC_STATS = 0x1000;
constexpr int PC_SPLIT = 0x2000;
constexpr int PC_FUSE  = 0x20000;
constexpr int PC_RLDS  = 0x40000;
constexpr int PC_SGATE = 0x80000;
constexpr int PC_BRELU = 0x100000;
constexpr int PC_UP4   = 0x200000;
constexpr int PC_ROWP  = 0x400000;
constexpr int PC_PSH   = 0x800000;
constexpr int PC_PRELU = 0x1000000;

constexpr int PC_BELOW_FUSE  = PC_FUSE - 1;
constexpr int PC_BELOW_RLDS  = PC_RLDS - 1;
constexpr int PC_BELOW_SGATE = PC_SGATE - 1;
constexpr int PC_BELOW_UP4   = PC_UP4 - 1;
```

innfer_amd/csrc/conv3x3_pc_loaders.inc:

```
    if (wave >= NCW) {
#if defined(__HIP_DEVICE_COMPILE__)
#ifdef INNFER_PRIO
        __builtin_amdgcn_s_setprio(INNFER_PRIO);
#else
        if constexpr (NT <= 2) __builtin_amdgcn_s_setprio(3);
#endif
#endif
        const int lw = wave - NCW;
        int loff[KQ];
        int lpix[POLY ? KQ : 1];
        int s9_ty0 = 0, s9_tx0 = 0, s9_n = 0; bool s9_edge = false;
        constexpr bool S2PRE = S2 && RPW == 2;
        int s2_off[S2PRE ? KQ : 1]; unsigned s2_m0 = 0, s2_m1 = 0, s2_m2 = 0, s2_m3 = 0;
        static_assert(!S2 || KQ <= 32, "one validity bit per piece");
        {
            const int ypar = p.up ? ((p.y0 - 1) & 1) : 0;
#pragma unroll
            for (int k = 0; k < KQ; ++k) {
                const int px = (lw + NLW * k) * 16 + (lane >> 2);
                const int ly = px / LWP;
                int lx = px - ly * LWP;
                const bool imgb = PAIR && lx >= 18;
                if (imgb) lx -= 18;
                const int slot = (lane & 3) ^ (((px >> 2) & 1) << 1);
                const int ry = S2 ? 2 * ly : p.up ? (ly + ypar) >> 1 : ly;
                const int rx = S2 ? 2 * lx : p.up ? (lx + 1) >> 1 : lx;
                constexpr int R0 = (TM & 0x007) ? 0 : (TM & 0x038) ? 1 : 2, R1 = (TM & 0x1C0) ? 2 : (TM & 0x038) ? 1 : 0;
                constexpr int S0 = (TM & 0x049) ? 0 : (TM & 0x092) ? 1 : 2, S1 = (TM & 0x124) ? 2 : (TM & 0x092) ? 1 : 0;
                const bool used = ly >= R0 && ly <= TH - 1 + R1 && lx >= S0 && lx <= TWI - 1 + S1;
                loff[k] = (px < NPX && lx < LVALID && used) ? ((ry * p.Ws + rx) * 32 + slot * 8) * 2 + (imgb ? (int)p.in_img_stride * 2 : 0) : OOB;
                if constexpr (POLY) {
                    lpix[k] = (px < NPX && lx < LVALID) ? (ly * p.fullW + lx) * 64 : -1;
                    loff[k] = slot * 16;
                }
            }
        }
        const int wvoff = lane * 16;
        int voff[KQ];
        const char* in_tile = nullptr;
        const char* w_tile = nullptr;
        auto setup = [&](int jj) __attribute__((always_inline)) {
            int kg, n, ty0, tx0, dl = 1;
            if constexpr (POLY) decode_poly(jj, kg, n, ty0, tx0, dl);
            else decode(jj, kg, n, ty0, tx0);
            const long n0 = PAIR ? 2L * n : n;
            const bool no_b = PAIR && 2 * n + 1 >= p.N;
            in_tile = (const char*)(p.in + n0 * p.in_img_stride) + ((long)((ty0 - 1) >> p.up) * p.Ws + ((tx0 >> p.up) - 1)) * 64;
            w_tile = (const char*)p.wpk + (long)kg * p.nchunks * W_BYTES;
#pragma unroll
            for (int k = 0; k < KQ; ++k) voff[k] = loff[k];
            if constexpr (POLY) {
                const int d = dl, dd = d * d;
                const int nn = n / dd, ph = n - nn * dd, py = ph / d, px = ph - py * d;
                const int Hp = (p.fullH - py + d - 1) / d, Wp = (p.fullW - px + d - 1) / d;
                in_tile = (const char*)(p.in + (long)nn * p.in_img_stride) + (((long)(ty0 - 1) * d + py) * p.fullW + (long)(tx0 - 1) * d + px) * 64;
                const bool edge = ty0 == 0 || ty0 + TH + 1 > Hp || tx0 == 0 || tx0 + TW + 1 > Wp;
#pragma unroll
                for (int k = 0; k < KQ; ++k) {
// ... 279 lines not shown
```

innfer_amd/csrc/conv3x3_pc_tile_end.inc:

```
            if constexpr (OUTMODE == OUT_SLAB && SPLIT) {
#define EPI(A, B, C) epilogue_slab_split<RPW, NT, A, B, C, CV>(p, acc, n, ty0, tx0, cw, li, cbase)
            if (!p.res1) {
                if (p.act == 1) EPI(1, false, false); else if (p.act == 2) EPI(2, false, false); else EPI(0, false, false);
            } else if (!p.res2) {
                if (p.act == 1) EPI(1, true, false); else if (p.act == 2) EPI(2, true, false);
                else if (NT == 2 && TM == TAPS_1X1 && p.act == 4) EPI((NT == 2 && TM == TAPS_1X1) ? 4 : 0, true, false);
                else if (NT == 2 && TM == TAPS_1X1 && p.act == 5) EPI((NT == 2 && TM == TAPS_1X1) ? 5 : 0, true, false);
                else EPI(0, true, false);
            } else {
                if (p.act == 1) EPI(1, true, true); else if (p.act == 2) EPI(2, true, true); else EPI(0, true, true);
            }
#undef EPI
            } else if constexpr (OUTMODE == OUT_SLAB && CV && RLDS) {
                if (p.res2) epilogue_slab_cv<RPW, NT, 0, false, true, true, ROWP>(p, acc, ty0, tx0, cw, li, cbase);
                else epilogue_slab_cv<RPW, NT, 0, false, false, true, ROWP>(p, acc, ty0, tx0, cw, li, cbase);
            } else if constexpr (OUTMODE == OUT_SLAB && RLDS) {
                if (p.res2) epilogue_slab<RPW, NT, 0, false, true, true, false, false, false, true, ROWP>(p, acc, n, ty0, tx0, cw, li, cbase, dcur);
                else epilogue_slab<RPW, NT, 0, false, false, true, false, false, false, true, ROWP>(p, acc, n, ty0, tx0, cw, li, cbase, dcur);
            } else if constexpr (OUTMODE == OUT_SLAB && CV) {
#define EPI(A, B, C) epilogue_slab_cv<RPW, NT, A, B, C, false, ROWP>(p, acc, ty0, tx0, cw, li, cbase)
            if (!p.res1) {
                if (p.act == 1) EPI(1, false, false); else if (p.act == 2) EPI(2, false, false);
                else if (NT == 4 && !ROWP && p.act == 7) EPI((NT == 4 && !ROWP) ? 7 : 0, false, false); else EPI(0, false, false);
            } else if (!p.res2) {
                if (p.act == 1) EPI(1, true, false); else if (p.act == 2) EPI(2, true, false); else EPI(0, true, false);
            } else {
                if (p.act == 1) EPI(1, true, true); else if (p.act == 2) EPI(2, true, true); else EPI(0, true, true);
            }
#undef EPI
            } else if constexpr (FUSE) {
                const int lidf = run_start + (p.rev ? run_len - 1 - (jt - slots) : (jt - slots));
                fused_last_epilogue<RPW, NT>(p, acc, smem + ((g & 1) * STAGE), smem + L::TAIL, n, ty0, tx0, cw, lane, lidf);
            } else if constexpr (PRELU) {
                f32x4 slope_r[NT];
#pragma unroll
                for (int t = 0; t < NT; ++t) slope_r[t] = *(const f32x4*)(slope_lds + lane_cbase<NT, ROWP>(lg) + toff_lin<NT, ROWP>(t));
                epilogue_slab<RPW, NT, 8, false, false, true, false, false, false, false, ROWP, false>(p, acc, n, ty0, tx0, cw, li, cbase, dcur, slope_r);
            } else if constexpr (OUTMODE == OUT_SLAB) {
            if constexpr (STATS) {
                const int lid = run_start + (p.rev ? run_len - 1 - (jt - slots) : (jt - slots));
                epilogue_stats<RPW, NT, TM == TAPS_PHASE, PAIR, NCW>(p, acc, bias_r, ty0, tx0, cw, li, cbase, lid / p.KG);
            }
#define EPI(A, B, C) epilogue_slab<RPW, NT, A, B, C, !(C), POLY, TM == TAPS_PHASE, PAIR, false, ROWP, PSH>(p, acc, n, ty0, tx0, cw, li, cbase, dcur)
            if (!p.res1) {
                if (p.act == 1) EPI(1, false, false); else if (p.act == 2) EPI(2, false, false);
                else if (NT == 4 && TM == TAPS_3X3 && !POLY && !ROWP && p.act == 7) EPI((NT == 4 && TM == TAPS_3X3 && !POLY && !ROWP) ? 7 : 0, false, false); else EPI(0, false, false);
            } else if (!p.res2) {
                if (p.act == 1) EPI(1, true, false); else if (p.act == 2) EPI(2, true, false); else if (p.act == 4) EPI(4, true, false);
                else if (p.act == 5) EPI(5, true, false); else EPI(0, true, false);
            } else {
                if (p.act == 1) EPI(1, true, true); else if (p.act == 2) EPI(2, true, true); else EPI(0, true, true);
            }
#undef EPI
// ... 4 lines not shown
```

innfer_amd/csrc/conv3x3_stats_gate_rlds.h:

```cpp

template <int RPW, int NT, bool DCV, bool PAIR, int NCW>
__device__ __forceinline__ void epilogue_stats(const KP& p, const f32x4 (&acc)[NT][2 * RPW], const f32x4 (&bias)[NT], int ty0, int tx0, int wave, int li,
                                               int cbase, int tile) {
    static_assert(NT == 4, "sixteen channels per lane: one per pixel lane after the transposing reduction");
    constexpr int MT = 2 * RPW;
    int yw = ty0 + wave * RPW, x0 = tx0, ylim = p.y1, c0 = cbase, slot = tile, ph = 0;
    if constexpr (DCV) {
        ph = cbase / p.phase_c;
        yw -= ph >> 1; x0 -= ph & 1; ylim = p.H;
        c0 -= ph * p.phase_c;
        slot = tile * 4 + ph;
    }
#pragma unroll
    for (int sg = 0; sg < (PAIR ? 2 : 1); ++sg) {
    if constexpr (PAIR) {
        const int q = tile / p.tiles_y, ty = tile - q * p.tiles_y;
        if (2 * q + sg >= p.N) continue;
        slot = (2 * q + sg) * p.tiles_y + ty;
        if constexpr (DCV) slot = slot * 4 + ph;
    }
    bool ok[MT];
#pragma unroll
    for (int m = 0; m < MT; ++m)
        ok[m] = PAIR ? ((m & 1) == sg && yw + (m >> 1) < ylim && x0 + li < p.W) : ((yw + (m >> 1) < ylim) && (x0 + li + (m & 1) * 16 < p.W));
// ... 52 lines not shown
    }
}

template <int MT>
__device__ __forceinline__ void self_gate_split(f32x4 (&acc)[2][MT], const f16x8* wh, const f16x8* wl, const f32x4* sgb) {
    const f32x4 z4 = {0.f, 0.f, 0.f, 0.f};
#pragma unroll
    for (int m = 0; m < MT; ++m) {
        f16x8 vh, vl;
#pragma unroll
        for (int t = 0; t < 2; ++t)
#pragma unroll
            for (int j = 0; j < 4; ++j) {
                const float f = acc[t][m][j];
                const f16 h = (f16)f;
                vh[4 * t + j] = h;
                vl[4 * t + j] = (f16)((f - (float)h) * 2048.0f);
            }
#pragma unroll
        for (int t = 0; t < 2; ++t) {
            const f32x4 gm = __builtin_amdgcn_mfma_f32_16x16x32_f16(wh[t], vh, sgb[t], 0, 0, 0);
            f32x4 gx = __builtin_amdgcn_mfma_f32_16x16x32_f16(wl[t], vh, z4, 0, 0, 0);
            gx = __builtin_amdgcn_mfma_f32_16x16x32_f16(wh[t], vl, gx, 0, 0, 0);
#pragma unroll
            for (int j = 0; j < 4; ++j) acc[t][m][j] = acc[t][m][j] * __builtin_amdgcn_rcpf(1.0f + __expf(-__builtin_fmaf(gx[j], 1.0f / 2048.0f, gm[j])));
        }
    }
}

template <int MT>
__device__ __forceinline__ void residual_from_lds(f32x4 (&acc)[4][MT], const char* st, const int* roffs, float rs1) {
#pragma unroll
    for (int m = 0; m < MT; ++m) {
        const f16x8 x0 = *(const f16x8*)(st + roffs[m]), x1 = *(const f16x8*)(st + roffs[m] + 16);
#pragma unroll
        for (int t = 0; t < 4; ++t)
#pragma unroll
            for (int j = 0; j < 4; ++j)
                acc[t][m][j] = __builtin_fmaf((float)(t < 2 ? x0 : x1)[(t & 1) * 4 + j], rs1, acc[t][m][j]);
    }
}

template <int MT, int HALF>
__device__ __forceinline__ void residual_from_lds_plane(f32x4 (&acc)[4][MT], const char* st, const int* roffs, float rs1) {
#pragma unroll
    for (int m = 0; m < MT; ++m) {
        const f16x8 x = *(const f16x8*)(st + roffs[m]);
#pragma unroll
        for (int tt = 0; tt < 2; ++tt)
#pragma unroll
            for (int j = 0; j < 4; ++j) acc[2 * HALF + tt][m][j] = __builtin_fmaf((float)x[tt * 4 + j], rs1, acc[2 * HALF + tt][m][j]);
    }
}
```

innfer_amd/csrc/net.hip:

```cpp
#include "common.h"
#include "norm_stats.h"

#include <cmath>
#include <cstring>
#include <mutex>

namespace innfer {

static thread_local std::string g_err;

int set_error(int code, const char* fmt, ...) {
    char buf[512];
    va_list ap;
    va_start(ap, fmt);
    vsnprintf(buf, sizeof buf, fmt, ap);
    va_end(ap);
    g_err = buf;
    return code;
}

namespace {
struct GtRec { std::string name; hipEvent_t e0, e1; double flops, bytes; };
thread_local std::vector<GtRec>* g_gt = nullptr;
thread_local hipEvent_t g_gt_e0 = nullptr;
// ... 52 lines not shown
#define INNFER_FUSE_LAST 1
#endif
struct ConvSlot {
    std::string key;
    int K = 0, C = 0;
    bool first = false;
    int ksize = 3;
    void* d_w = nullptr;
    std::vector<float> h_w;
    void* d_w32 = nullptr;
    bool rowp = false;
    bool up2x = false;
    void* d_up4 = nullptr;
    void* d_up4p = nullptr;
    float* d_b4 = nullptr;
    bool ps2 = false;
    void* d_ps = nullptr;
    float* d_bps = nullptr;
    void* d_fuse = nullptr;
    float* d_b = nullptr;
    int Kp = 0;
    bool slope_ok = false;
    float* d_slope = nullptr;
    bool loaded = false;
    bool map_ok = false;
    float* d_map = nullptr;
    int map_act = 0;
};

struct innfer_net {
    int kind = 0;
    int in_nc = 3, out_nc = 3, nf = 64, nb = 23, gc = 32, scale = 4, n_up = 2;
    int final_act = 0;
    int band_rows = 0;
    int nr = 3;
    int trunk_act = 1;
    bool ps_up = false;
    float res_scale = 1.f;
    int outm = 0;
    int u8_normalize = 0, u8_round16 = 1;
#ifndef INNFER_UP_PHASES_DEFAULT
#define INNFER_UP_PHASES_DEFAULT 1
#endif
    int up_phases = INNFER_UP_PHASES_DEFAULT;
    int fused_tail = 1;
#ifndef INNFER_HR_CHAIN_DEFAULT
#define INNFER_HR_CHAIN_DEFAULT 1
#endif
    int hr_chain = INNFER_HR_CHAIN_DEFAULT;
#ifndef INNFER_PS_PC_DEFAULT
#define INNFER_PS_PC_DEFAULT 1
#endif
    int ps_pc = INNFER_PS_PC_DEFAULT;
    int res_lds = 1;
    bool plus = false;
    int unshuffle = 1;
    int fp32 = 0;
    std::vector<ConvSlot> convs;
};

static int n_upscale(int scale) {
    if (scale == 3) return 1;
    int n = 0;
    while ((1 << n) < scale) ++n;
    return n;
}

static void add_conv(innfer_net* net, const std::string& key, int K, int C, bool first = false, int ksize = 3) {
    ConvSlot s;
    s.key = key; s.K = K; s.C = C; s.first = first; s.ksize = ksize;
    net->convs.push_back(s);
}

extern "C" int innfer_version(void) { return INNFER_ABI_VERSION; }
extern "C" const char* innfer_last_error(void) { return g_err.c_str(); }

extern "C" int innfer_rrdbnet_create(innfer_net_t* out, int in_nc, int out_nc, int nf, int nb,
                                     int gc, int scale, int plus) {
    return innfer_rrdbnet_create_ex(out, in_nc, out_nc, nf, nb, gc, scale, plus, 3, 1, 0);
}

extern "C" int innfer_rrdbnet_create_ex(innfer_net_t* out, int in_nc, int out_nc, int nf, int nb,
                                        int gc, int scale, int plus, int nr, int act, int pixelshuffle_up) {
    return innfer_rrdbnet_create_ex2(out, in_nc, out_nc, nf, nb, gc, scale, plus, nr, act, pixelshuffle_up, 1);
}

extern "C" int innfer_rrdbnet_create_ex2(innfer_net_t* out, int in_nc, int out_nc, int nf, int nb,
                                         int gc, int scale, int plus, int nr, int act, int pixelshuffle_up, int unshuffle) {
    if (!out) return set_error(INNFER_ERR_INVALID, "rrdbnet_create: null out");
    if (nr < 1 || nr > 64 || (act != 1 && act != 2))
        return set_error(INNFER_ERR_UNSUPPORTED, "rrdbnet_create: nr=%d act=%d (built: nr >= 1; act 1 LeakyReLU(0.2), 2 ReLU)", nr, act);
    if (pixelshuffle_up && scale == 3 && nf != 64)
        return set_error(INNFER_ERR_UNSUPPORTED, "rrdbnet_create: PixelShuffle(3) is built for nf=64 (nf %d: 9 nf is not a multiple of 64)", nf);
    if (scale != 1 && scale != 2 && scale != 3 && scale != 4 && scale != 8 && scale != 16)
        return set_error(INNFER_ERR_UNSUPPORTED, "rrdbnet_create: scale %d (built: 1, 2, 3, 4, 8, 16)", scale);
    if (nf % 32 || gc % 32 || nf <= 0 || gc <= 0 || nf > 64)
        return set_error(INNFER_ERR_UNSUPPORTED, "rrdbnet_create: nf=%d gc=%d (need nf in {32,64}, gc %% 32 == 0)", nf, gc);
    if (in_nc < 1 || in_nc > 8 || out_nc < 1 || out_nc > 16 || nb < 1)
        return set_error(INNFER_ERR_INVALID, "rrdbnet_create: in_nc=%d out_nc=%d nb=%d", in_nc, out_nc, nb);
    if (unshuffle != 1 && unshuffle != 2 && unshuffle != 4)
        return set_error(INNFER_ERR_UNSUPPORTED, "rrdbnet_create: unshuffle %d (built: 1, 2, 4)", unshuffle);
    if (unshuffle > 1 && in_nc != 3)
        return set_error(INNFER_ERR_UNSUPPORTED, "rrdbnet_create: unshuffle %d with in_nc=%d (the folded pixel_unshuffle is built for in_nc 3: 12 or 48 channels into the first conv)", unshuffle, in_nc);
    innfer_net* net = new innfer_net();
    net->unshuffle = unshuffle;
    net->kind = 0; net->in_nc = in_nc; net->out_nc = out_nc; net->nf = nf; net->nb = nb;
// ... 231 lines not shown
        if (c.d_map) { (void)hipFree(c.d_map); c.d_map = nullptr; }
        c.map_act = 0;
        return INNFER_OK;
    }
    if (!c.map_ok)
        return set_error(INNFER_ERR_UNSUPPORTED, "set_conv_input_map: '%s' (built in front of the first conv of an SRResNet block and of LR_conv of either network)", c.key.c_str());
    std::vector<float> h(2 * (size_t)c.C);
    for (int i = 0; i < c.C; ++i) { h[i] = alpha ? alpha[i] : 1.f; h[c.C + i] = shift ? shift[i] : 0.f; }
    if (!c.d_map) INNFER_HIP(hipMalloc((void**)&c.d_map, h.size() * sizeof(float)));
    INNFER_HIP(hipMemcpy(c.d_map, h.data(), h.size() * sizeof(float), hipMemcpyHostToDevice));
    c.map_act = act;
    return INNFER_OK;
}

extern "C" int innfer_net_set_precision(innfer_net_t net, int fp32) {
    if (!net || (fp32 != 0 && fp32 != 1)) return set_error(INNFER_ERR_INVALID, "set_precision: 0 (fp16 arithmetic) or 1 (fp32-accurate)");
    if (fp32 && net->kind == 2) return set_error(INNFER_ERR_UNSUPPORTED, "set_precision: SRVGGNetCompact is built for the fp16 mode only (no fp32-accurate engine)");
    if (fp32) {
        std::vector<ConvSlot*> built;
        for (auto& c : net->convs) {
            if (c.first || c.d_w32 || !c.loaded) continue;
            const int rc = build_split_panels(c);
            if (rc != INNFER_OK) {
                for (ConvSlot* q : built) { (void)hipFree(q->d_w32); q->d_w32 = nullptr; }
                return rc;
            }
            built.push_back(&c);
        }
    }
    net->fp32 = fp32;
    return INNFER_OK;
}

extern "C" int innfer_net_set_band_rows(innfer_net_t net, int rows) {
    if (!net || rows < 0) return set_error(INNFER_ERR_INVALID, "set_band_rows: bad arguments");
    net->band_rows = rows;
    return INNFER_OK;
}

extern "C" int innfer_net_set_upconv_phases(innfer_net_t net, int on) {
    if (!net) return set_error(INNFER_ERR_INVALID, "set_upconv_phases: null network");
    if (on < 0 || on > 2) return set_error(INNFER_ERR_INVALID, "set_upconv_phases: 0 (nine taps on the HR grid), 1 (four phases, one visit of a tile: default) or 2 (one phase per visit)");
    net->up_phases = on;
    return INNFER_OK;
}

extern "C" int innfer_net_set_residual_lds(innfer_net_t net, int on) {
    if (!net) return set_error(INNFER_ERR_INVALID, "set_residual_lds: null network");
    if (on < 0 || on > 2) return set_error(INNFER_ERR_INVALID, "set_residual_lds: 0 (epilogue loads), 1 (the RRDB-end layers: default) or 2 (every dense block)");
    net->res_lds = on;
    return INNFER_OK;
}

extern "C" int innfer_net_set_fused_tail(innfer_net_t net, int on) {
    if (!net) return set_error(INNFER_ERR_INVALID, "set_fused_tail: null network");
    net->fused_tail = on ? 1 : 0;
    return INNFER_OK;
}

extern "C" int innfer_net_set_hr_chain(innfer_net_t net, int on) {
    if (!net) return set_error(INNFER_ERR_INVALID, "set_hr_chain: null network");
    net->hr_chain = on ? 1 : 0;
    return INNFER_OK;
}

extern "C" int innfer_net_set_u8_io(innfer_net_t net, int normalize, int fp16_mode) {
    if (!net) return set_error(INNFER_ERR_INVALID, "set_u8_io: null net");
    net->u8_normalize = normalize != 0;
    net->u8_round16 = fp16_mode != 0;
    return INNFER_OK;
}

extern "C" int innfer_net_set_final_act(innfer_net_t net, int act) {
    if (!net || (act != 0 && act != 1 && act != 2 && act != 3 && act != 6))
        return set_error(INNFER_ERR_INVALID, "set_final_act: act %d (0 none, 1 LeakyReLU(0.2), 2 ReLU, 3 tanh, 6 sigmoid)", act);
    net->final_act = act;
    return INNFER_OK;
}

extern "C" double innfer_net_flops(innfer_net_t net, int N, int H, int W) {
    if (!net) return 0.0;
    H = (H + net->unshuffle - 1) / net->unshuffle; W = (W + net->unshuffle - 1) / net->unshuffle;
    double px = (double)N * H * W, f = 0.0;
    const int nconv = (int)net->convs.size();
    for (int i = 0; i < nconv; ++i) {
        const ConvSlot& c = net->convs[i];
        double mult = 1.0;
        const int tail0 = nconv - 2 - net->n_up;
        if (i >= tail0) {
            const int u = i - tail0;
            const double f2 = net->scale == 3 ? 9.0 : 4.0;
            if (u < net->n_up) mult = std::pow(f2, !net->ps_up ? u + 1 : u);
            else mult = std::pow(f2, net->n_up);
        }
        f += 2.0 * c.ksize * c.ksize * c.K * c.C * px * mult;
    }
    return f;
}

struct Carve {
    size_t fea, slab[3], trunk, up[5], hr, tmp, total;
    size_t lo;
    int slab_w;
};

static Carve carve(const innfer_net* net, int N, int H, int W) {
// ... 275 lines not shown
    return timed_end(s, px * k, px * (k * 2.0 + net->in_nc * (T.base_u8 ? 1.0 : 2.0) + k * (T.out_mode == 2 ? 1.0 : T.out_mode == 1 ? 4.0 : 2.0)), 6000);
}

int run_chain(std::vector<ConvLaunch>& chain, int band_rows, hipStream_t s) {
    if (chain.empty()) return INNFER_OK;
    const int H = chain[0].H, L = (int)chain.size();
    if (band_rows <= 0 || band_rows >= H) {
        for (auto& c : chain) { int rc = do_conv(c, s); if (rc) return rc; }
        return INNFER_OK;
    }
    const int nbands = (H + (L - 1) + band_rows - 1) / band_rows;
    for (int b = 0; b < nbands; ++b)
        for (int l = 0; l < L; ++l) {
            int y0 = b * band_rows - l, y1 = y0 + band_rows;
            if (y0 < 0) y0 = 0;
            if (y1 > H) y1 = H;
            if (b == nbands - 1) y1 = H;
            if (y0 >= y1) continue;
            ConvLaunch c = chain[l];
            c.y0 = y0; c.y1 = y1;
            int rc = do_conv(c, s);
            if (rc) return rc;
        }
    return INNFER_OK;
}

}

extern "C" int innfer_net_forward(innfer_net_t net, const void* d_in, int in_dtype, void* d_out, int out_dtype,
                                  int N, int H, int W, void* d_ws, size_t ws_bytes, void* stream) {
    if (!net || !d_in || !d_out || !d_ws) return set_error(INNFER_ERR_INVALID, "forward: null argument");
    if (N <= 0 || H <= 0 || W <= 0) return set_error(INNFER_ERR_INVALID, "forward: bad shape %dx%dx%d", N, H, W);
    auto dtype_ok = [](int d) { return d == INNFER_F16 || d == INNFER_F32 || d == INNFER_U8; };
    if (!dtype_ok(in_dtype) || !dtype_ok(out_dtype)) return set_error(INNFER_ERR_INVALID, "forward: bad dtype");
    if (out_dtype == INNFER_U8 && net->out_nc > 4) return set_error(INNFER_ERR_UNSUPPORTED, "forward: a uint8 image has at most 4 channels (out_nc %d)", net->out_nc);
    for (auto& c : net->convs)
        if (!c.loaded) return set_error(INNFER_ERR_INVALID, "forward: weights of '%s' were never set", c.key.c_str());
    const int img_h = H, img_w = W;
    H = (H + net->unshuffle - 1) / net->unshuffle; W = (W + net->unshuffle - 1) / net->unshuffle;
    const Carve cv = carve(net, N, H, W);
    if (ws_bytes < cv.total) return set_error(INNFER_ERR_WORKSPACE, "forward: workspace %zu < %zu bytes", ws_bytes, cv.total);
    hipStream_t s = (hipStream_t)stream;
    char* ws = (char*)d_ws;
    if (net->kind == 2) return compact_forward(net, d_in, in_dtype, d_out, out_dtype, N, H, W, ws, cv, s);
    const int nf = net->nf, gc = net->gc;
    const long G = (long)N * H * W * 32;
    const long LO = (long)(cv.lo / 2);
    if (net->fp32) {
        if (in_dtype == INNFER_F16) return set_error(INNFER_ERR_INVALID, "forward: the fp32-accurate mode takes fp32 or uint8 input (an fp16 tensor is the fp16 mode's)");
        for (auto& c : net->convs)
            if (!c.first && !c.d_w32) return set_error(INNFER_ERR_INVALID, "forward: the fp32-accurate panels of '%s' are missing: call innfer_net_set_precision(net, 1) after the last innfer_net_set_conv", c.key.c_str());
    }
    auto mk = [&](const ConvSlot& cs, const f16* in, long in_g, void* out, long out_g, int N_, int H_, int W_, int act) {
        return mk_launch(cs, in, in_g, out, out_g, N_, H_, W_, act, LO);
    };
    f16* fea = (f16*)(ws + cv.fea);
    f16* slab[3] = {(f16*)(ws + cv.slab[0]), (f16*)(ws + cv.slab[1]), (f16*)(ws + cv.slab[2])};
    f16* trunk = (f16*)(ws + cv.trunk);
    int ci = 0;

    if (net->unshuffle > 1) {
        const ConvSlot& c0 = net->convs[ci++];
        FirstUnshuffleLaunch F{};
        F.in = d_in; F.in_f32 = in_dtype == INNFER_F32; F.Cin = net->in_nc; F.r = net->unshuffle; F.wpk = c0.d_w; F.bias = c0.d_b;
        F.in_u8 = in_dtype == INNFER_U8; F.in_norm = net->u8_normalize; F.in_round16 = net->u8_round16;
        F.out = fea; F.out_gstride = G; F.out2 = slab[0]; F.out2_gstride = G;
        F.K = nf; F.N = N; F.H = img_h; F.W = img_w; F.act = 0;
        F.out_lo = LO; F.out2_lo = LO;
        int rc = do_first_unshuffle(F, s);
        if (rc) return rc;
    } else {
        const ConvSlot& c0 = net->convs[ci++];
        FirstConvLaunch F{};
        F.in = d_in; F.in_f32 = in_dtype == INNFER_F32; F.Cin = c0.C; F.w = (const float*)c0.d_w; F.bias = c0.d_b;
        F.in_u8 = in_dtype == INNFER_U8; F.in_norm = net->u8_normalize; F.in_round16 = net->u8_round16;
        F.out = fea; F.out_gstride = G; F.out2 = slab[0]; F.out2_gstride = G;
        if (net->kind == 1 && net->nb > 0) F.out2 = nullptr;
        F.K = nf; F.N = N; F.H = H; F.W = W; F.act = 0;
        F.out_lo = LO; F.out2_lo = LO;
        int rc = do_first(F, s);
        if (rc) return rc;
    }

    std::vector<ConvLaunch> chain;
    int cur = 0;
    if (net->kind == 0) {
        for (int b = 0; b < net->nb; ++b) {
            const int in_slab = cur;
            const int f1 = (cur + 1) % 3, f2 = (cur + 2) % 3;
            const int nr = net->nr;
            int last = in_slab;
            for (int r = 0; r < nr; ++r) {
                const int work_r = last, dest_r = (r == 0 || last == f2) ? f1 : f2;
                last = dest_r;
                f16* S = slab[work_r];
                f16* t1x1 = (f16*)(ws + cv.tmp);
                if (net->plus) {
                    const ConvSlot& cs = net->convs[ci++];
                    chain.push_back(mk(cs, S, G, t1x1, G, N, H, W, 0));
                }
                for (int i = 0; i < 4; ++i) {
                    const ConvSlot& cs = net->convs[ci++];
                    ConvLaunch L = mk(cs, S, G, S + (long)((nf + i * gc) / 32) * G, G, N, H, W, net->trunk_act);
                    if (net->plus && i == 1) { L.res1 = t1x1; L.res1_gstride = G; L.s1 = 1.f; }
                    if (net->plus && i == 3) {
                        L.res1 = S + (long)((nf + gc) / 32) * G; L.res1_gstride = G; L.s1 = 1.f;
                    }
// ... 253 lines not shown
    return INNFER_OK;
}
extern "C" int innfer_pack_selfgate(const float* w32x32, void* packed_2k) {
    if (!w32x32 || !packed_2k) return set_error(INNFER_ERR_INVALID, "pack_selfgate: null argument");
    conv_pack_selfgate(w32x32, packed_2k);
    return INNFER_OK;
}
extern "C" size_t innfer_conv7x7_packed_bytes(int K, int C) { return (K > 0 && C > 0 && C % 32 == 0) ? conv_packed_bytes7x7(K, C) : 0; }
extern "C" int innfer_pack_conv7x7(const float* w, int K, int C, void* packed) {
    if (!w || !packed || K <= 0 || C <= 0 || C % 32) return set_error(INNFER_ERR_INVALID, "pack_conv7x7: K=%d C=%d (%% 32)", K, C);
    conv_pack7x7(w, K, C, packed);
    return INNFER_OK;
}
extern "C" int innfer_pack_up2x_phases(const float* w, int K, int C, int plane_rows, void* packed) {
    if (!w || !packed || K <= 0 || K % 64 || C <= 0 || C % 32) return set_error(INNFER_ERR_INVALID, "pack_up2x_phases: K=%d (%% 64) C=%d (%% 32)", K, C);
    conv_pack_up2x_phases(w, K, C, packed, plane_rows ? 1 : 0);
    return INNFER_OK;
}

static int conv_args_stats(const innfer_conv_args* a, int phases, ConvLaunch& L) {
    if (!a->d_stats_part) return INNFER_OK;
    if (a->N <= 0 || a->H <= 0 || a->W <= 0 || a->K <= 0) return set_error(INNFER_ERR_INVALID, "conv3x3: statistics of an empty launch (N=%d H=%d W=%d K=%d)", a->N, a->H, a->W, a->K);
    const long long need = (long long)a->N * conv_stats_nper(a->H, a->W, phases) * a->K * 3;
    if ((long long)a->stats_part_floats < need)
        return set_error(INNFER_ERR_WORKSPACE, "conv3x3: stats_part_floats %lld < %lld (N * records * channels * 3)", (long long)a->stats_part_floats, need);
    L.stats_part = a->d_stats_part;
    return INNFER_OK;
}

extern "C" int innfer_conv_stats_records(int H, int W, int phases) {
    if (H <= 0 || W <= 0 || (phases != 1 && phases != 4)) return set_error(INNFER_ERR_INVALID, "conv_stats_records: H=%d W=%d phases=%d (1 | 4)", H, W, phases);
    return conv_stats_nper(H, W, phases);
}

extern "C" int innfer_norm_combine_parts(const float* d_part, int nper, int64_t HW, float eps, const float* d_gamma, const float* d_beta, float* d_alpha, float* d_shift,
                                         int C, int N, void* stream) {
    if (!d_part || !d_alpha || !d_shift || nper <= 0 || HW <= 0 || C <= 0 || N <= 0 || N > 65535)
        return set_error(INNFER_ERR_INVALID, "norm_combine_parts: null argument or nper=%d HW=%lld C=%d N=%d", nper, (long long)HW, C, N);
    return norm::launch_combine_parts(d_part, nper, (long)HW, eps, d_gamma, d_beta, d_alpha, d_shift, C, N, (hipStream_t)stream);
}

extern "C" int innfer_norm_stats(const void* d_src, int slab, int64_t gs, int cpad, int64_t HW, float eps, const float* d_gamma, const float* d_beta, float* d_alpha,
                                 float* d_shift, int C, int N, float* d_part, int64_t part_floats, void* stream) {
    if (!d_src || !d_alpha || !d_shift || HW <= 0 || C <= 0 || N <= 0 || N > 65535 || (HW + norm::SEG - 1) / norm::SEG > 65535)
        return set_error(INNFER_ERR_INVALID, "norm_stats: null argument or HW=%lld C=%d N=%d", (long long)HW, C, N);
    if (slab ? gs < (int64_t)N * HW * 32 : (cpad < C || cpad % 32))
        return set_error(INNFER_ERR_INVALID, "norm_stats: group stride %lld < N * HW * 32 (slab), or cpad=%d below C=%d / not a multiple of 32 (fp32)", (long long)gs, cpad, C);
    if (HW > norm::SEG && (!d_part || part_floats < 0 || (unsigned long long)part_floats < (unsigned long long)N * norm::part_floats(C, (long)HW)))
        return set_error(INNFER_ERR_WORKSPACE, "norm_stats: part_floats %lld < %llu", (long long)part_floats, (unsigned long long)N * norm::part_floats(C, (long)HW));
    return slab ? norm::launch_stats_slab((const f16*)d_src, (long)gs, (long)HW, eps, d_gamma, d_beta, d_alpha, d_shift, C, N, d_part, (hipStream_t)stream)
                : norm::launch_stats((const float*)d_src, cpad, (long)HW, eps, d_gamma, d_beta, d_alpha, d_shift, C, N, d_part, (hipStream_t)stream);
}

static int conv3x3_f16_impl(const innfer_conv_args* a, const float* d_slope, void* stream);
extern "C" int innfer_conv3x3_f16(const innfer_conv_args* a, void* stream) { return conv3x3_f16_impl(a, nullptr, stream); }
extern "C" int innfer_conv3x3_f16_slope(const innfer_conv_args* a, const float* d_slope, void* stream) { return conv3x3_f16_impl(a, d_slope, stream); }

extern "C" int innfer_shuffle_add(const void* d_slab, int64_t group_stride, const void* d_base, int base_dtype, int normalize, void* d_out, int out_dtype,
                                  int N, int C, int H, int W, int scale, void* stream) {
    if ((base_dtype != INNFER_F16 && base_dtype != INNFER_U8) || (out_dtype != INNFER_F16 && out_dtype != INNFER_F32 && out_dtype != INNFER_U8))
        return set_error(INNFER_ERR_UNSUPPORTED, "shuffle_add: base fp16 or uint8, result fp16, fp32 or uint8");
    ShuffleAddLaunch T{};
    T.slab = (const f16*)d_slab; T.gstride = group_stride;
    T.base = d_base; T.base_u8 = base_dtype == INNFER_U8; T.base_norm = normalize != 0;
    T.out = d_out; T.out_mode = out_dtype == INNFER_U8 ? 2 : out_dtype == INNFER_F32 ? 1 : 0; T.out_denorm = normalize != 0;
    T.C = C; T.s = scale; T.N = N; T.H = H; T.W = W;
    return shuffle_add_launch(T, (hipStream_t)stream);
}

static int conv3x3_f16_impl(const innfer_conv_args* a, const float* d_slope, void* stream) {
    if (!a || !a->d_in || !a->d_packed || !a->d_bias || !a->d_out) return set_error(INNFER_ERR_INVALID, "conv3x3: null argument");
    const bool forms121 = a->conv1x1 || a->prefix_lrelu || a->d_gate_packed || a->d_gate_bias || a->in_relu || a->conv7x7 || a->out_planar || a->out_denorm || a->out_round16 ||
                          a->planar_phases || a->outm;
    if (forms121 && (a->column7 || a->stride2_k4 || a->transposed2x || a->pixel_shuffle2 || a->dilation > 1 || a->dilation_groups || a->d_stats_part))
        return set_error(INNFER_ERR_UNSUPPORTED, "conv3x3: conv1x1 / prefix_lrelu / the self gate / in_relu / conv7x7 / out_planar / planar_phases / outm do not combine with "
                                                 "column7 / stride2_k4 / transposed2x / pixel_shuffle2 / dilation / d_stats_part");
    if ((a->act == 3 || a->act == 6) && !a->out_planar) return set_error(INNFER_ERR_INVALID, "conv3x3: act %d (tanh / sigmoid) is an activation of planar outputs (out_planar)", a->act);
    if (a->out_planar < 0 || a->out_planar > 3 || (!a->out_planar && (a->out_denorm || a->out_round16 || a->planar_phases)) || ((a->out_denorm || a->out_round16) && a->out_planar != 3))
        return set_error(INNFER_ERR_INVALID, "conv3x3: out_planar=%d (0..3); planar_phases needs out_planar, out_denorm / out_round16 the uint8 image (3)", a->out_planar);
    if (a->prefix_lrelu && !a->conv1x1) return set_error(INNFER_ERR_INVALID, "conv3x3: prefix_lrelu is an operand form of conv1x1");
    if ((a->d_gate_packed != nullptr) != (a->d_gate_bias != nullptr)) return set_error(INNFER_ERR_INVALID, "conv3x3: the self gate takes d_gate_packed and d_gate_bias");
    if (a->conv7x7 && !a->out_planar) return set_error(INNFER_ERR_UNSUPPORTED, "conv7x7: planar output (out_planar) with K <= 16 only");
    if (a->column7) {
        if (a->K <= 0 || a->K % 32 || a->K > 64 || a->out_ch_off || a->row_begin || a->row_end || a->dilation > 1 || a->dilation_groups || a->pixel_shuffle2 ||
            a->upsample2x || a->d_res1 || a->d_res2 || a->stride2_k4 || a->transposed2x || a->act < 0 || a->act > 2)
            return set_error(INNFER_ERR_UNSUPPORTED, "conv7x1: K %% 32 == 0, K <= 64 (K=%d), act 0..2, all rows, no residual / upsampling", a->K);
        ConvLaunch L{};
        L.in = (const f16*)a->d_in; L.in_gstride = a->in_group_stride; L.C = a->C;
        L.wpk = (const f16*)a->d_packed; L.bias = a->d_bias;
        L.out = a->d_out; L.out_gstride = a->out_group_stride; L.K = a->K;
        L.N = a->N; L.H = a->H; L.W = a->W; L.act = a->act; L.s1 = L.s2 = 1.f; L.y0 = 0; L.y1 = a->H; L.out_mode = OUT_SLAB;
        L.conv7v = 1; L.reflect = a->reflect_pad ? 1 : 0;
        if (int rc = conv_args_stats(a, 1, L)) return rc;
        return conv_launch(L, (hipStream_t)stream);
    }
    if (a->stride2_k4 || a->transposed2x) {
        if ((a->stride2_k4 && a->transposed2x) || (a->transposed2x && a->transposed2x != 3 && a->transposed2x != 4) || a->K <= 0 || a->K % 64 || a->out_ch_off ||
            a->row_begin || a->row_end || a->dilation > 1 || a->dilation_groups || a->reflect_pad || a->pixel_shuffle2 || a->upsample2x || a->d_res1 || a->d_res2 ||
            a->act < 0 || a->act > 2)
            return set_error(INNFER_ERR_UNSUPPORTED, "conv: the stride-2 forms need K %% 64 == 0 (K=%d), act 0..2, all rows, zero padding, no residual / upsampling", a->K);
        ConvLaunch L{};
        L.in = (const f16*)a->d_in; L.in_gstride = a->in_group_stride; L.C = a->C;
        L.wpk = (const f16*)a->d_packed; L.bias = a->d_bias;
        L.out = a->d_out; L.out_gstride = a->out_group_stride; L.K = a->K;
        L.N = a->N; L.H = a->H; L.W = a->W; L.act = a->act; L.s1 = L.s2 = 1.f; L.y0 = 0; L.y1 = a->H; L.out_mode = OUT_SLAB;
        if (a->stride2_k4) L.stride2 = 1;
        else { L.K = 4 * a->K; L.phase_c = a->K; L.deconv_phases = 1; L.rowp = a->plane_rows ? 1 : 0; }
        if (int rc = conv_args_stats(a, a->stride2_k4 ? 1 : 4, L)) return rc;
        return conv_launch(L, (hipStream_t)stream);
    }
    const int Kl = a->planar_phases ? 4 * a->K : a->K;
    if (a->out_planar) {
        if (a->K <= 0 || a->K > 64 || Kl > 64 || a->out_ch_off)
            return set_error(INNFER_ERR_UNSUPPORTED, "conv3x3: a planar output holds 1 .. 64 channels (K=%d%s) at out_ch_off 0", a->K, a->planar_phases ? ", four phases each" : "");
    } else if (a->pixel_shuffle2) {
        if (a->K <= 0 || a->K % 64 || a->out_ch_off || a->row_begin || a->row_end || a->dilation > 1 || a->dilation_groups || a->reflect_pad || a->act < 0 || a->act > 2)
            return set_error(INNFER_ERR_UNSUPPORTED, "conv3x3: the PixelShuffle(2) store needs K %% 64 == 0 (K=%d), out_ch_off 0, act 0..2, all rows, plain zero padding", a->K);
    } else if (a->dilation_groups > 0 ? a->K != 32 * a->dilation_groups : (a->K <= 0 || a->K % 16 || (a->K > 64 && !(a->d_stats_part && a->K % 64 == 0))))
        return set_error(INNFER_ERR_UNSUPPORTED, "conv3x3: K=%d (need K %% 16 == 0, K <= 64 -- with d_stats_part any K %% 64 == 0; K = 32 * dilation_groups)", a->K);
    ConvLaunch L{};
    if (a->out_ch_off % 16 || (a->out_ch_off % 32 && a->K > 16))
        return set_error(INNFER_ERR_INVALID, "conv3x3: out_ch_off=%d must keep the %d output channels inside 32-channel groups", a->out_ch_off, a->K);
    L.in = (const f16*)a->d_in; L.in_gstride = a->in_group_stride; L.C = a->C;
    L.wpk = (const f16*)a->d_packed; L.bias = a->d_bias;
    L.out = (f16*)a->d_out + (long)(a->out_ch_off / 32) * a->out_group_stride; L.out_gstride = a->out_group_stride;
    L.out_coff = a->out_ch_off % 32; L.K = a->K;
    L.N = a->N; L.H = a->H; L.W = a->W; L.act = a->act; L.up = a->upsample2x;
    L.res1 = (const f16*)a->d_res1; L.res1_gstride = a->res1_group_stride; L.s1 = a->res1_scale;
    L.res2 = (const f16*)a->d_res2; L.res2_gstride = a->res2_group_stride; L.s2 = a->res2_scale;
    L.y0 = a->row_begin; L.y1 = a->row_end > 0 ? a->row_end : a->H;
    L.out_mode = a->pixel_shuffle2 ? OUT_SHUFFLE2 : OUT_SLAB; L.reflect = a->reflect_pad; L.dilation = a->dilation; L.dilation_groups = a->dilation_groups;
    L.res1_lds = a->res1_from_input ? 2 : 0;
    L.slope = d_slope;
    L.rowp = a->plane_rows ? 1 : 0;
    if (a->pixel_shuffle2 && a->plane_rows == 2) L.rowp = 2;
    else if (a->pixel_shuffle2 && a->plane_rows) return set_error(INNFER_ERR_INVALID, "conv3x3: pixel_shuffle2 takes plane_rows 0 (innfer_pack_conv3x3 panels) or 2 (innfer_pack_conv3x3_shuffle2 panels)");
    if (a->reserved0) return set_error(INNFER_ERR_UNSUPPORTED, "conv3x3: innfer_conv_args.reserved0 (the row-Winograd experiment until ABI 111) must be 0");
    L.conv1x1 = a->conv1x1 ? 1 : 0; L.prefix_lrelu = a->prefix_lrelu ? 1 : 0; L.in_relu = a->in_relu ? 1 : 0; L.conv7 = a->conv7x7 ? 1 : 0;
    L.gate_w = (const f16*)a->d_gate_packed; L.gate_bias = a->d_gate_bias;
    L.outm = a->outm;
    if (a->out_planar) {
        L.out = a->d_out; L.out_coff = 0; L.K = Kl; L.out_mode = OUT_NCHW;
        L.out_f32 = a->out_planar == 2; L.out_u8 = a->out_planar == 3; L.out_denorm = a->out_denorm ? 1 : 0; L.out_round16 = a->out_round16 ? 1 : 0;
        L.phase_c = a->planar_phases ? a->K : 0;
    }
    if (a->split) {
        if (a->pixel_shuffle2 || (!a->out_planar && (a->K % 32 || a->out_lo <= 0)) || a->in_lo <= 0 || (a->d_res1 && a->res1_lo <= 0) || (a->d_res2 && a->res2_lo <= 0))
            return set_error(INNFER_ERR_UNSUPPORTED, "conv3x3 (split): K in {32, 64} (K=%d), slab output, the lo distances of every tensor given", a->K);
        L.split = 1; L.in_lo = a->in_lo; L.out_lo = a->out_lo; L.res1_lo = a->res1_lo; L.res2_lo = a->res2_lo;
    }
    if (int rc = conv_args_stats(a, 1, L)) return rc;
    return conv_launch(L, (hipStream_t)stream);
}

extern "C" int innfer_nchw_to_slab(const void* d_src, int src_dtype, void* d_slab, int64_t group_stride, int ch_off,
                                   int N, int C, int H, int W, void* stream) {
    return nchw_to_slab(d_src, src_dtype == INNFER_F32, (f16*)d_slab, group_stride, ch_off, N, C, H, W, (hipStream_t)stream);
}

extern "C" int innfer_slab_to_nchw(const void* d_slab, int64_t group_stride, int ch_off, void* d_dst, int dst_dtype,
                                   int N, int C, int H, int W, void* stream) {
    return slab_to_nchw((const f16*)d_slab, group_stride, ch_off, d_dst, dst_dtype == INNFER_F32, N, C, H, W, (hipStream_t)stream);
}

extern "C" int innfer_first_conv_unshuffle(const void* d_in, int in_dtype, int normalize, int fp16_mode, int N, int in_nc, int H, int W, int unshuffle,
                                           const float* h_weight_oihw, const float* h_bias, int K, int act, void* d_slab, int64_t group_stride, int64_t lo, void* stream) {
    if (!d_in || !h_weight_oihw || !d_slab) return set_error(INNFER_ERR_INVALID, "first_conv_unshuffle: null argument");
    if (in_dtype != INNFER_F16 && in_dtype != INNFER_F32 && in_dtype != INNFER_U8) return set_error(INNFER_ERR_INVALID, "first_conv_unshuffle: bad dtype");
    if ((unshuffle != 2 && unshuffle != 4) || in_nc != 3 || (K != 32 && K != 64) || act < 0 || act > 2 || N <= 0 || H <= 0 || W <= 0)
        return set_error(INNFER_ERR_UNSUPPORTED, "first_conv_unshuffle: unshuffle %d (2 | 4), in_nc %d (3), K %d (32 | 64), act %d (0..2)", unshuffle, in_nc, K, act);
    const long px = (long)N * ((H + unshuffle - 1) / unshuffle) * ((W + unshuffle - 1) / unshuffle);
    if (group_stride < px * 32 || lo < 0) return set_error(INNFER_ERR_INVALID, "first_conv_unshuffle: group_stride %ld < %ld", (long)group_stride, px * 32);
    std::vector<char> host(first_unshuffle_packed_bytes(K, unshuffle));
    first_unshuffle_pack(h_weight_oihw, K, unshuffle, host.data());
    std::vector<float> bias(K, 0.f);
    if (h_bias) for (int k = 0; k < K; ++k) bias[k] = h_bias[k];
    void* d_w = nullptr; float* d_b = nullptr;
    INNFER_HIP(hipMalloc(&d_w, host.size()));
    if (hipMalloc((void**)&d_b, K * sizeof(float)) != hipSuccess) { (void)hipFree(d_w); return set_error(INNFER_ERR_NOMEM, "first_conv_unshuffle: out of device memory"); }
    int rc = INNFER_OK;
    if (hipMemcpy(d_w, host.data(), host.size(), hipMemcpyHostToDevice) != hipSuccess || hipMemcpy(d_b, bias.data(), K * sizeof(float), hipMemcpyHostToDevice) != hipSuccess)
        rc = set_error(INNFER_ERR_HIP, "first_conv_unshuffle: copying the weights failed");
    if (rc == INNFER_OK) {
        FirstUnshuffleLaunch F{};
        F.in = d_in; F.in_f32 = in_dtype == INNFER_F32; F.Cin = in_nc; F.in_u8 = in_dtype == INNFER_U8; F.in_norm = normalize != 0; F.in_round16 = fp16_mode != 0;
        F.r = unshuffle; F.wpk = d_w; F.bias = d_b; F.out = (f16*)d_slab; F.out_gstride = group_stride; F.K = K; F.N = N; F.H = H; F.W = W; F.act = act; F.out_lo = lo;
// ... 7 lines not shown
```

innfer_amd/lib.py:

```python
import ctypes as C
import os

_HERE = os.path.dirname(os.path.abspath(__file__))
_DEFAULT_LIB = os.path.join(_HERE, "lib", "libinnfer_amd.so")
LIB_PATH = os.environ.get("INNFER_LIB") or _DEFAULT_LIB

F16, F32, U8 = 0, 1, 2
OK, ERR_INVALID, ERR_HIP, ERR_UNSUPPORTED, ERR_NOMEM, ERR_WORKSPACE = 0, -1, -2, -3, -4, -5


class InnferError(RuntimeError):
    pass


def _load():
    if not os.path.isfile(LIB_PATH):
        raise ImportError(
            f"{LIB_PATH} not found: build it with `make` (or `python -c 'import __graft_entry__ as g; g.build()'`). "
            "innfer_amd has no CPU or PyTorch fallback for its hot path.")
    import torch
    return C.CDLL(LIB_PATH)


_lib = _load()
# ... 37 lines not shown
        ("phase_k", C.c_int),
        ("form", C.c_int),
    ]


class GatherGemmArgs(C.Structure):
    _fields_ = [
        ("d_in", C.c_void_p), ("in_group_stride", C.c_int64), ("cin_pad", C.c_int),
        ("d_packed", C.c_void_p), ("cout_pad", C.c_int),
        ("d_raw", C.c_void_p), ("raw_stride", C.c_int), ("cout_store", C.c_int),
        ("N", C.c_int), ("Hin", C.c_int), ("Win", C.c_int), ("Ho", C.c_int), ("Wo", C.c_int), ("stride", C.c_int),
        ("ntaps", C.c_int), ("dy", C.c_int * 49), ("dx", C.c_int * 49),
        ("Hfull", C.c_int), ("Wfull", C.c_int), ("os", C.c_int), ("ooy", C.c_int), ("oox", C.c_int), ("up", C.c_int), ("reflect", C.c_int),
        ("ngroup", C.c_int), ("g_wbytes", C.c_int64), ("g_outoff", C.c_int64), ("g_tapmul", C.c_int), ("g_phase", C.c_int),
        ("d_scratch", C.c_void_p), ("scratch_bytes", C.c_int64),
        ("keep_partials", C.c_int),
    ]


SIGNATURES = {
    "innfer_version": (C.c_int, []),
    "innfer_last_error": (C.c_char_p, []),
    "innfer_rrdbnet_create": (C.c_int, [C.POINTER(C.c_void_p)] + [C.c_int] * 7),
    "innfer_srresnet_create": (C.c_int, [C.POINTER(C.c_void_p)] + [C.c_int] * 5),
    "innfer_net_destroy": (None, [C.c_void_p]),
    "innfer_net_num_convs": (C.c_int, [C.c_void_p]),
    "innfer_net_conv_info": (C.c_int, [C.c_void_p, C.c_int, C.c_char_p, C.c_size_t,
                                       C.POINTER(C.c_int), C.POINTER(C.c_int)]),
    "innfer_net_set_conv": (C.c_int, [C.c_void_p, C.c_int, C.c_void_p, C.c_void_p]),
    "innfer_net_scale": (C.c_int, [C.c_void_p]),
    "innfer_net_workspace_bytes": (C.c_size_t, [C.c_void_p, C.c_int, C.c_int, C.c_int]),
    "innfer_net_forward": (C.c_int, [C.c_void_p, C.c_void_p, C.c_int, C.c_void_p, C.c_int,
                                     C.c_int, C.c_int, C.c_int, C.c_void_p, C.c_size_t, C.c_void_p]),
    "innfer_net_forward_timed": (C.c_int, [C.c_void_p, C.c_void_p, C.c_int, C.c_void_p, C.c_int,
                                           C.c_int, C.c_int, C.c_int, C.c_void_p, C.c_size_t, C.c_void_p,
                                           C.c_int, C.POINTER(C.c_float), C.POINTER(C.c_double), C.POINTER(C.c_double),
                                           C.POINTER(C.c_int), C.POINTER(C.c_int)]),
    "innfer_rrdbnet_create_ex": (C.c_int, [C.POINTER(C.c_void_p)] + [C.c_int] * 10),
    "innfer_rrdbnet_create_ex2": (C.c_int, [C.POINTER(C.c_void_p)] + [C.c_int] * 11),
    "innfer_first_conv_unshuffle": (C.c_int, [C.c_void_p] + [C.c_int] * 8 + [C.c_void_p, C.c_void_p, C.c_int, C.c_int, C.c_void_p, C.c_int64, C.c_int64, C.c_void_p]),
    "innfer_srresnet_create_ex": (C.c_int, [C.POINTER(C.c_void_p)] + [C.c_int] * 6 + [C.c_float, C.c_int]),
    "innfer_net_set_conv_input_map": (C.c_int, [C.c_void_p, C.c_int, C.c_void_p, C.c_void_p, C.c_int]),
    "innfer_net_set_outm": (C.c_int, [C.c_void_p, C.c_int]),
    "innfer_timer_start": (C.c_int, []),
    "innfer_timer_stop": (C.c_int, [C.c_void_p, C.c_int, C.c_char_p, C.c_int, C.POINTER(C.c_float), C.POINTER(C.c_double), C.POINTER(C.c_double), C.POINTER(C.c_int)]),
    "innfer_net_set_precision": (C.c_int, [C.c_void_p, C.c_int]),
    "innfer_pack_conv3x3_split": (C.c_int, [C.c_void_p, C.c_int, C.c_int, C.c_void_p]),
    "innfer_nchw_to_slab_split": (C.c_int, [C.c_void_p, C.c_void_p, C.c_int64, C.c_int64] + [C.c_int] * 5 + [C.c_void_p]),
    "innfer_slab_split_to_nchw": (C.c_int, [C.c_void_p, C.c_int64, C.c_int64, C.c_int, C.c_void_p] + [C.c_int] * 4 + [C.c_void_p]),
    "innfer_net_set_band_rows": (C.c_int, [C.c_void_p, C.c_int]),
    "innfer_net_set_fused_tail": (C.c_int, [C.c_void_p, C.c_int]),
    "innfer_net_set_hr_chain": (C.c_int, [C.c_void_p, C.c_int]),
    "innfer_net_set_residual_lds": (C.c_int, [C.c_void_p, C.c_int]),
    "innfer_net_set_upconv_phases": (C.c_int, [C.c_void_p, C.c_int]),
    "innfer_net_set_final_act": (C.c_int, [C.c_void_p, C.c_int]),
    "innfer_net_flops": (C.c_double, [C.c_void_p, C.c_int, C.c_int, C.c_int]),
    "innfer_unet_create": (C.c_int, [C.POINTER(C.c_void_p), C.c_int, C.c_int, C.c_int, C.c_int]),
    "innfer_unet_create_ex": (C.c_int, [C.POINTER(C.c_void_p)] + [C.c_int] * 6),
    "innfer_unet_destroy": (None, [C.c_void_p]),
    "innfer_unet_num_params": (C.c_int, [C.c_void_p]),
    "innfer_unet_param_info": (C.c_int, [C.c_void_p, C.c_int, C.c_char_p, C.c_size_t, C.POINTER(C.c_int), C.POINTER(C.c_int)]),
    "innfer_unet_set_param": (C.c_int, [C.c_void_p, C.c_int, C.c_void_p]),
    "innfer_unet_set_eval": (C.c_int, [C.c_void_p, C.c_int]),
    "innfer_unet_set_precision": (C.c_int, [C.c_void_p, C.c_int]),
    "innfer_unet_workspace_bytes": (C.c_size_t, [C.c_void_p, C.c_int, C.c_int, C.c_int]),
    "innfer_unet_flops": (C.c_double, [C.c_void_p, C.c_int, C.c_int, C.c_int]),
    "innfer_unet_forward": (C.c_int, [C.c_void_p, C.c_void_p, C.c_int, C.c_void_p, C.c_int,
                                      C.c_int, C.c_int, C.c_int, C.c_void_p, C.c_size_t, C.c_void_p]),
    "innfer_pan_create": (C.c_int, [C.POINTER(C.c_void_p), C.c_int, C.c_int, C.c_int, C.c_int, C.c_int, C.c_int]),
    "innfer_pan_create_ex": (C.c_int, [C.POINTER(C.c_void_p)] + [C.c_int] * 9),
    "innfer_pan_destroy": (None, [C.c_void_p]),
    "innfer_pan_num_params": (C.c_int, [C.c_void_p]),
    "innfer_pan_param_info": (C.c_int, [C.c_void_p, C.c_int, C.c_char_p, C.c_size_t, C.POINTER(C.c_int), C.POINTER(C.c_int)]),
    "innfer_pan_set_param": (C.c_int, [C.c_void_p, C.c_int, C.c_void_p]),
    "innfer_pan_set_fused_scpa": (C.c_int, [C.c_void_p, C.c_int]),
    "innfer_pan_set_precision": (C.c_int, [C.c_void_p, C.c_int]),
    "innfer_pan_workspace_bytes": (C.c_size_t, [C.c_void_p, C.c_int, C.c_int, C.c_int]),
    "innfer_pan_forward": (C.c_int, [C.c_void_p, C.c_void_p, C.c_int, C.c_void_p, C.c_int,
                                     C.c_int, C.c_int, C.c_int, C.c_void_p, C.c_size_t, C.c_void_p]),
    "innfer_ppon_create": (C.c_int, [C.POINTER(C.c_void_p), C.c_int, C.c_int, C.c_int, C.c_int, C.c_int, C.c_float]),
    "innfer_ppon_destroy": (None, [C.c_void_p]),
    "innfer_ppon_num_params": (C.c_int, [C.c_void_p]),
    "innfer_ppon_param_info": (C.c_int, [C.c_void_p, C.c_int, C.c_char_p, C.c_size_t, C.POINTER(C.c_int), C.POINTER(C.c_int)]),
    "innfer_ppon_set_precision": (C.c_int, [C.c_void_p, C.c_int]),
    "innfer_ppon_set_param": (C.c_int, [C.c_void_p, C.c_int, C.c_void_p]),
    "innfer_ppon_workspace_bytes": (C.c_size_t, [C.c_void_p, C.c_int, C.c_int, C.c_int]),
    "innfer_ppon_forward": (C.c_int, [C.c_void_p, C.c_void_p, C.c_int, C.c_void_p, C.c_void_p, C.c_void_p, C.c_int,
                                      C.c_int, C.c_int, C.c_int, C.c_void_p, C.c_size_t, C.c_void_p]),
    "innfer_resnet_create": (C.c_int, [C.POINTER(C.c_void_p), C.c_int, C.c_int, C.c_int, C.c_int]),
    "innfer_resnet_create_ex": (C.c_int, [C.POINTER(C.c_void_p)] + [C.c_int] * 8),
    "innfer_resnet_set_eval": (C.c_int, [C.c_void_p, C.c_int]),
    "innfer_resnet_destroy": (None, [C.c_void_p]),
    "innfer_resnet_num_params": (C.c_int, [C.c_void_p]),
    "innfer_resnet_param_info": (C.c_int, [C.c_void_p, C.c_int, C.c_char_p, C.c_size_t, C.POINTER(C.c_int), C.POINTER(C.c_int)]),
    "innfer_resnet_set_precision": (C.c_int, [C.c_void_p, C.c_int]),
    "innfer_resnet_set_param": (C.c_int, [C.c_void_p, C.c_int, C.c_void_p]),
    "innfer_resnet_workspace_bytes": (C.c_size_t, [C.c_void_p, C.c_int, C.c_int, C.c_int]),
    "innfer_resnet_forward": (C.c_int, [C.c_void_p, C.c_void_p, C.c_int, C.c_void_p, C.c_int,
                                        C.c_int, C.c_int, C.c_int, C.c_void_p, C.c_size_t, C.c_void_p]),
    "innfer_wbc_create": (C.c_int, [C.POINTER(C.c_void_p), C.c_int, C.c_int]),
    "innfer_wbc_destroy": (None, [C.c_void_p]),
    "innfer_wbc_num_params": (C.c_int, [C.c_void_p]),
    "innfer_wbc_param_info": (C.c_int, [C.c_void_p, C.c_int, C.c_char_p, C.c_size_t, C.POINTER(C.c_int), C.POINTER(C.c_int)]),
    "innfer_wbc_set_precision": (C.c_int, [C.c_void_p, C.c_int]),
    "innfer_wbc_set_param": (C.c_int, [C.c_void_p, C.c_int, C.c_void_p]),
    "innfer_wbc_workspace_bytes": (C.c_size_t, [C.c_void_p, C.c_int, C.c_int, C.c_int]),
    "innfer_wbc_forward": (C.c_int, [C.c_void_p, C.c_void_p, C.c_int, C.c_void_p, C.c_int,
                                     C.c_int, C.c_int, C.c_int, C.c_void_p, C.c_size_t, C.c_void_p]),
    "innfer_guided_filter_workspace_bytes": (C.c_size_t, [C.c_int, C.c_int, C.c_int, C.c_int]),
    "innfer_guided_filter": (C.c_int, [C.c_void_p, C.c_void_p, C.c_int, C.c_int, C.c_int, C.c_int, C.c_int, C.c_float, C.c_void_p,
                                       C.c_void_p, C.c_size_t, C.c_void_p]),
    "innfer_conv3x3_packed_bytes": (C.c_size_t, [C.c_int, C.c_int]),
    "innfer_pack_conv3x3": (C.c_int, [C.c_void_p, C.c_int, C.c_int, C.c_void_p]),
    "innfer_pack_conv3x3_rows": (C.c_int, [C.c_void_p, C.c_int, C.c_int, C.c_int, C.c_void_p]),
    "innfer_pack_conv3x3_shuffle2": (C.c_int, [C.c_void_p, C.c_void_p, C.c_int, C.c_int, C.c_void_p, C.c_void_p]),
    "innfer_pack_convt2x_rows": (C.c_int, [C.c_void_p, C.c_int, C.c_int, C.c_int, C.c_int, C.c_void_p]),
    "innfer_conv3x3_f16": (C.c_int, [C.POINTER(ConvArgs), C.c_void_p]),
    "innfer_conv3x3_f16_slope": (C.c_int, [C.POINTER(ConvArgs), C.c_void_p, C.c_void_p]),
    "innfer_shuffle_add": (C.c_int, [C.c_void_p, C.c_int64, C.c_void_p, C.c_int, C.c_int, C.c_void_p, C.c_int] + [C.c_int] * 5 + [C.c_void_p]),
    "innfer_compact_create": (C.c_int, [C.POINTER(C.c_void_p)] + [C.c_int] * 5),
    "innfer_net_set_conv_slope": (C.c_int, [C.c_void_p, C.c_int, C.c_void_p]),
    "innfer_conv1x1_packed_bytes": (C.c_size_t, [C.c_int, C.c_int]),
    "innfer_pack_conv1x1": (C.c_int, [C.c_void_p, C.c_int, C.c_int, C.c_void_p]),
    "innfer_pack_conv1x1_split": (C.c_int, [C.c_void_p, C.c_int, C.c_int, C.c_void_p]),
    "innfer_pack_selfgate": (C.c_int, [C.c_void_p, C.c_void_p]),
    "innfer_conv7x7_packed_bytes": (C.c_size_t, [C.c_int, C.c_int]),
    "innfer_pack_conv7x7": (C.c_int, [C.c_void_p, C.c_int, C.c_int, C.c_void_p]),
    "innfer_pack_up2x_phases": (C.c_int, [C.c_void_p, C.c_int, C.c_int, C.c_int, C.c_void_p]),
    "innfer_filter2d": (C.c_int, [C.c_void_p, C.c_int, C.c_long, C.c_int, C.c_int, C.c_void_p, C.c_int, C.c_int, C.c_int, C.c_int, C.c_int, C.c_void_p, C.c_void_p]),
    "innfer_conv7x1_packed_bytes": (C.c_size_t, [C.c_int, C.c_int]),
    "innfer_pack_conv7x1": (C.c_int, [C.c_void_p, C.c_int, C.c_int, C.c_void_p]),
    "innfer_conv4x4s2_packed_bytes": (C.c_size_t, [C.c_int, C.c_int]),
    "innfer_pack_conv4x4s2": (C.c_int, [C.c_void_p, C.c_int, C.c_int, C.c_void_p]),
    "innfer_convt2x_packed_bytes": (C.c_size_t, [C.c_int, C.c_int]),
    "innfer_pack_convt2x": (C.c_int, [C.c_void_p, C.c_int, C.c_int, C.c_int, C.c_void_p]),
    "innfer_nchw_to_slab": (C.c_int, [C.c_void_p, C.c_int, C.c_void_p, C.c_int64, C.c_int,
                                      C.c_int, C.c_int, C.c_int, C.c_int, C.c_void_p]),
    "innfer_slab_to_nchw": (C.c_int, [C.c_void_p, C.c_int64, C.c_int, C.c_void_p, C.c_int,
                                      C.c_int, C.c_int, C.c_int, C.c_int, C.c_void_p]),
    "innfer_chop_plan": (C.c_int, [C.c_int, C.c_int, C.c_int, C.c_double, C.POINTER(C.c_int),
                                   C.POINTER(C.c_int), C.POINTER(C.c_int), C.POINTER(C.c_int),
                                   C.POINTER(C.c_int)]),
    "innfer_extract_tiles": (C.c_int, [C.c_void_p, C.c_int, C.c_int, C.c_int, C.c_int, C.c_int, C.c_double,
                                       C.c_int, C.c_int, C.c_void_p, C.c_void_p]),
    "innfer_blend_profile": (C.c_int, [C.c_int, C.c_double, C.c_int, C.POINTER(C.c_float)]),
    "innfer_recompose": (C.c_int, [C.c_void_p, C.c_int, C.c_int, C.c_int, C.c_int, C.c_int, C.c_int,
                                   C.c_double, C.c_int, C.c_void_p, C.c_int, C.c_void_p]),
    "innfer_shard_tiles": (C.c_int, [C.c_int, C.c_int, C.c_int, C.POINTER(C.c_int), C.POINTER(C.c_int)]),
    "innfer_comm_unique_id": (C.c_int, [C.c_void_p]),
    "innfer_comm_init": (C.c_int, [C.POINTER(C.c_void_p), C.c_void_p, C.c_int, C.c_int]),
    "innfer_comm_destroy": (None, [C.c_void_p]),
    "innfer_comm_rank": (C.c_int, [C.c_void_p]),
    "innfer_comm_size": (C.c_int, [C.c_void_p]),
    "innfer_gather_tiles": (C.c_int, [C.c_void_p, C.c_void_p, C.c_size_t, C.c_int, C.c_void_p]),
    "innfer_comm_broadcast": (C.c_int, [C.c_void_p, C.c_void_p, C.c_size_t, C.c_int, C.c_void_p]),
    "innfer_u8hwc_to_nchw": (C.c_int, [C.c_void_p, C.c_int, C.c_int, C.c_int, C.c_int, C.c_void_p, C.c_int, C.c_void_p]),
    "innfer_srgb_to_linear": (C.c_int, [C.c_void_p, C.c_void_p, C.c_size_t, C.c_void_p]),
    "innfer_linear_to_srgb": (C.c_int, [C.c_void_p, C.c_void_p, C.c_size_t, C.c_void_p]),
    "innfer_color_fix_workspace_bytes": (C.c_size_t, [C.c_int, C.c_int, C.c_int, C.c_int, C.c_int]),
    "innfer_color_fix": (C.c_int, [C.c_void_p, C.c_int, C.c_int, C.c_void_p, C.c_int, C.c_int, C.c_int, C.c_void_p,
                                   C.c_void_p, C.c_size_t, C.c_void_p]),
    "innfer_nchw_to_u8hwc": (C.c_int, [C.c_void_p, C.c_int, C.c_int, C.c_int, C.c_int, C.c_int, C.c_void_p, C.c_void_p]),
    "innfer_linear_resize": (C.c_int, [C.c_void_p, C.c_int, C.c_int, C.c_int, C.c_void_p, C.c_int, C.c_int, C.c_void_p, C.c_size_t, C.c_void_p]),
    "innfer_extract_tiles_u8": (C.c_int, [C.c_void_p, C.c_int, C.c_int, C.c_int, C.c_int, C.c_int, C.c_double, C.c_int, C.c_int, C.c_void_p, C.c_int, C.c_void_p]),
    "innfer_recompose_u8": (C.c_int, [C.c_void_p, C.c_int, C.c_int, C.c_int, C.c_int, C.c_int, C.c_int, C.c_double, C.c_int, C.c_int, C.c_int, C.c_void_p, C.c_void_p]),
    "innfer_net_set_u8_io": (C.c_int, [C.c_void_p, C.c_int, C.c_int]),
    "innfer_guided_filter_ex": (C.c_int, [C.c_void_p, C.c_void_p, C.c_int, C.c_int, C.c_int, C.c_int, C.c_int, C.c_int, C.c_float,
                                          C.c_void_p, C.c_int, C.c_int, C.c_void_p, C.c_void_p, C.c_size_t, C.c_void_p]),
    "innfer_inthwc_to_nchw": (C.c_int, [C.c_void_p, C.c_int, C.c_int, C.c_int, C.c_int, C.c_int, C.c_int, C.c_float, C.c_void_p, C.c_int, C.c_void_p]),
    "innfer_nchw_to_inthwc": (C.c_int, [C.c_void_p, C.c_int, C.c_int, C.c_int, C.c_int, C.c_int, C.c_int, C.c_int, C.c_void_p, C.c_void_p]),
    "innfer_channel_minmax": (C.c_int, [C.c_void_p] + [C.c_int] * 5 + [C.c_void_p, C.c_void_p]),
# ... 213 lines not shown
```

Baseline: 494.6 MPix/s.

## Add 2x4 consumer-wave grid for 64-channel slab conv with residual prefetch

```diff
diff --git a/include/innfer_amd.h b/include/innfer_amd.h
--- a/include/innfer_amd.h
+++ b/include/innfer_amd.h
@@ -68,6 +68,8 @@
 int innfer_net_set_band_rows(innfer_net_t net, int rows);
 
 int innfer_net_set_residual_lds(innfer_net_t net, int on);
+
+int innfer_net_set_consumer_grid(innfer_net_t net, int mode);
 
 int innfer_net_set_fused_tail(innfer_net_t net, int on);
 int innfer_net_set_hr_chain(innfer_net_t net, int on);
@@ -206,6 +208,7 @@
 int innfer_pack_up2x_phases(const float* h_weight_oihw, int K, int C, int plane_rows, void* h_packed);
 int innfer_conv3x3_f16(const innfer_conv_args* a, void* stream);
 int innfer_conv3x3_f16_slope(const innfer_conv_args* a, const float* d_slope, void* stream);
+int innfer_conv3x3_f16_grid(const innfer_conv_args* a, int consumer_grid, void* stream);
 int innfer_shuffle_add(const void* d_slab, int64_t group_stride, const void* d_base, int base_dtype, int normalize, void* d_out, int out_dtype,
                        int N, int C, int H, int W, int scale, void* stream);
 int innfer_pack_conv3x3_split(const float* h_weight_oihw, int K, int C, void* h_packed);
diff --git a/innfer_amd/architectures/engine_module.py b/innfer_amd/architectures/engine_module.py
--- a/innfer_amd/architectures/engine_module.py
+++ b/innfer_amd/architectures/engine_module.py
@@ -44,6 +44,7 @@
         self.upconv_phases = True
         self.hr_chain = True
         self.fused_tail = True
+        self.consumer_grid = 1
         self.residual_lds = 1
 
     unshuffle = 1
@@ -166,6 +167,8 @@
         L.check(L.lib.innfer_net_set_fused_tail(self._handle, int(bool(self.fused_tail))))
         L.check(L.lib.innfer_net_set_hr_chain(self._handle, int(bool(self.hr_chain))))
         L.check(L.lib.innfer_net_set_residual_lds(self._handle, int(self.residual_lds)))
+        if hasattr(L.lib, 'innfer_net_set_consumer_grid'):
+            L.check(L.lib.innfer_net_set_consumer_grid(self._handle, int(self.consumer_grid)))
         L.check(L.lib.innfer_net_set_upconv_phases(self._handle, int(self.upconv_phases)))
         L.check(L.lib.innfer_net_set_outm(self._handle, int(getattr(self, '_outm', 0))))
         L.check(L.lib.innfer_net_set_precision(self._handle, int(x.dtype == torch.float32)))
@@ -198,6 +201,8 @@
             L.check(L.lib.innfer_net_set_fused_tail(self._handle, int(bool(self.fused_tail))))
             L.check(L.lib.innfer_net_set_hr_chain(self._handle, int(bool(self.hr_chain))))
             L.check(L.lib.innfer_net_set_residual_lds(self._handle, int(self.residual_lds)))
+            if hasattr(L.lib, 'innfer_net_set_consumer_grid'):
+                L.check(L.lib.innfer_net_set_consumer_grid(self._handle, int(self.consumer_grid)))
             L.check(L.lib.innfer_net_set_upconv_phases(self._handle, int(self.upconv_phases)))
             L.check(L.lib.innfer_net_set_u8_io(self._handle, int(bool(normalize)), int(bool(fp16))))
             L.check(L.lib.innfer_net_set_precision(self._handle, int(not fp16)))
diff --git a/innfer_amd/csrc/common.h b/innfer_amd/csrc/common.h
--- a/innfer_amd/csrc/common.h
+++ b/innfer_amd/csrc/common.h
@@ -107,6 +107,7 @@
     const f16* gate_w; const float* gate_bias;
     const float* slope;
     int res1_lds;
+    int grid2;
 };
 
 int conv_nt_for(int K);
diff --git a/innfer_amd/csrc/conv3x3.hip b/innfer_amd/csrc/conv3x3.hip
--- a/innfer_amd/csrc/conv3x3.hip
+++ b/innfer_amd/csrc/conv3x3.hip
@@ -387,13 +387,16 @@
     constexpr bool SPLIT = (TMF & PC_SPLIT) != 0;
     static_assert(!SPLIT || (!S9 && !POLY && !S2 && !PFX && !STATS && (TM == TAPS_3X3 || TM == TAPS_1X1)), "split operands: plain 3x3 and 1x1 convs");
     constexpr bool RLDS = (TMF & PC_RLDS) != 0;
-    static_assert(!RLDS || (RPW == 2 && NT == 4 && NCW == 8 && NSI == 2 && OUTMODE == OUT_SLAB && (TMF & PC_BELOW_RLDS) == TAPS_3X3 && !S9 && !POLY), "residual from LDS: the plain 64-channel instantiation (and its canvas form)");
+    constexpr bool GRID2 = (TMF & PC_GRID2) != 0;
+    static_assert(!GRID2 || (RPW == 4 && NT == 2 && NCW == 8 && NSI == 2 && OUTMODE == OUT_SLAB && (TMF & ~(TAPS_3X3 | PC_RLDS | PC_ROWP | PC_GRID2)) == 0 && (TMF & PC_ROWP) && TM == TAPS_3X3 && !S9 && !POLY && !CV),
+                  "2 x 4 consumer grid: the plain and the RLDS 64-output plane-order slab conv");
+    static_assert(!RLDS || (((RPW == 2 && NT == 4) || GRID2) && NCW == 8 && NSI == 2 && OUTMODE == OUT_SLAB && (TMF & PC_BELOW_RLDS) == TAPS_3X3 && !S9 && !POLY), "residual from LDS: the plain 64-channel instantiation (its canvas form, its 2 x 4 consumer grid)");
     constexpr bool SGATE = (TMF & PC_SGATE) != 0;
     static_assert(!SGATE || (RPW == 3 && NT == 2 && NCW == 8 && OUTMODE == OUT_SLAB && ((TMF & PC_BELOW_SGATE) == TAPS_3X3 || (TMF & PC_BELOW_SGATE) == (TAPS_3X3 | PC_SPLIT)) && !S9 && !POLY), "self gate: the 32-output slab kernel (its canvas form, its split-operand form)");
     constexpr bool BRELU = (TMF & PC_BRELU) != 0;
     constexpr bool UP4 = (TMF & PC_UP4) != 0;
     constexpr bool ROWP = (TMF & PC_ROWP) != 0;
-    static_assert(!ROWP || (RPW == 2 && NT == 4 && NCW == 8 && OUTMODE == OUT_SLAB && TM == TAPS_3X3 && (TMF & ~(TAPS_3X3 | PC_FUSE | PC_RLDS | PC_UP4 | PC_ROWP | PC_PSH | PC_PRELU)) == 0 && !S9 && !POLY), "plane row order: the 64-channel slab kernels");
+    static_assert(!ROWP || (((RPW == 2 && NT == 4) || GRID2) && NCW == 8 && OUTMODE == OUT_SLAB && TM == TAPS_3X3 && (TMF & ~(TAPS_3X3 | PC_FUSE | PC_RLDS | PC_UP4 | PC_ROWP | PC_PSH | PC_PRELU | PC_GRID2)) == 0 && !S9 && !POLY), "plane row order: the 64-channel slab kernels");
     constexpr bool PSH = (TMF & PC_PSH) != 0;
     static_assert(!PSH || (ROWP && (TMF & ~(TAPS_3X3 | PC_ROWP | PC_PSH)) == 0 && NSI == 2 && !CV), "pixel-shuffle store: the plain 64-channel plane-order instantiation");
     static_assert(!UP4 || (RPW == 2 && NT == 4 && NCW == 8 && NSI == 3 && OUTMODE == OUT_SLAB && (TMF & PC_BELOW_UP4) == TAPS_3X3 && !S9 && !POLY && !CV), "one-pass phases: the 64-channel slab kernel on three input slots");
@@ -408,7 +411,7 @@
     constexpr int IN_BYTES = L::IN_BYTES;
     constexpr int NQ = IN_BYTES / 1024;
     constexpr int KQ = (NQ + NLW - 1) / NLW;
-    constexpr int WROWS = NT * 16;
+    constexpr int WROWS = L::WROWS;
     constexpr int NTAP = L::NTAP;
     constexpr int W_BYTES = L::W_BYTES;
     constexpr int WQ = W_BYTES / 1024;
@@ -475,13 +478,14 @@
     __builtin_amdgcn_s_setprio(INNFER_CPRIO);
 #endif
     const int cw = wave;
+    const int cwr = GRID2 ? (cw & 3) : cw;
     int boffs[3][2];
 #pragma unroll
     for (int s = 0; s < 3; ++s)
 #pragma unroll
         for (int par = 0; par < 2; ++par) {
-            const int pb = cw * RPW * LWP + li + s;
-            const int rowpar = ((cw * RPW) & 1) ^ par;
+            const int pb = cwr * RPW * LWP + li + s;
+            const int rowpar = ((cwr * RPW) & 1) ^ par;
             boffs[s][par] = pb * 64 + ((lg ^ (((((li + s) >> 2) & 1) ^ rowpar) << 1)) << 4);
         }
     int boffp[PAIR ? 3 : 1][2];
@@ -495,12 +499,16 @@
                 boffp[s][par] = pb * 64 + ((lg ^ (((((18 + li + s) >> 2) & 1) ^ rowpar) << 1)) << 4);
             }
     }
-    const int aoffs = li * 64 + ((lg ^ (((li >> 2) & 1) << 1)) << 4);
-    int roffs[RLDS ? MT : 1];
-    if constexpr (RLDS) {
+    const int aoffs = li * 64 + ((lg ^ (((li >> 2) & 1) << 1)) << 4) + (GRID2 ? (cw >> 2) * 32 * 64 : 0);
+    int roffs[RLDS ? (GRID2 ? 2 : MT) : 1];
+    if constexpr (RLDS && GRID2) {
+#pragma unroll
+        for (int par = 0; par < 2; ++par)
+            roffs[par] = ((cwr * RPW + 1) * LWP + li + 1) * 64 + ((lg ^ (((((li + 1) >> 2) & 1) ^ par) << 1)) << 4);
+    } else if constexpr (RLDS) {
 #pragma unroll
         for (int m = 0; m < MT; ++m) {
-            const int P = (cw * RPW + (m >> 1) + 1) * LWP + li + (m & 1) * 16 + 1;
+            const int P = (cwr * RPW + (m >> 1) + 1) * LWP + li + (m & 1) * 16 + 1;
             roffs[m] = P * 64 + (((lg & 1) ^ ((P >> 2) & 1)) << 5);
             if constexpr (ROWP) roffs[m] = P * 64 + ((lg ^ (((P >> 2) & 1) << 1)) << 4);
         }
@@ -570,6 +578,13 @@
         for (int e = 0; e < 8; ++e) pfx[m][e] = 0.f;
     int jt = j0, c = 0;
     int kg = 0, n = 0, ty0 = 0, tx0 = 0, cbase = 0, dcur = 1;
+    [[maybe_unused]] f16x4 rpre[GRID2 ? MT : 1][NT];
+    if constexpr (GRID2) {
+#pragma unroll
+        for (int m = 0; m < MT; ++m)
+#pragma unroll
+            for (int t = 0; t < NT; ++t) rpre[m][t] = f16x4{0, 0, 0, 0};
+    }
     asm volatile("s_barrier" ::: "memory");
 #ifdef INNFER_STAMPS
     const unsigned long long k_c0 = clock64(), k_w0 = wall_clock64();
@@ -578,7 +593,7 @@
         if (c == 0) {
             if constexpr (POLY) decode_poly(jt, kg, n, ty0, tx0, dcur);
             else decode(jt, kg, n, ty0, tx0);
-            cbase = kg * WROWS + lane_cbase<NT, ROWP>(lg);
+            cbase = kg * WROWS + (GRID2 ? (cw >> 2) * 32 : 0) + lane_cbase<NT, ROWP>(lg);
             if (kg != bias_kg) {
 #pragma unroll
                 for (int t = 0; t < NT; ++t) bias_r[t] = *(const f32x4*)(p.bias + cbase + toff_lin<NT, ROWP>(t));
@@ -599,6 +614,14 @@
                         for (int j = 0; j < 4; ++j) acc[t][m][j] = __builtin_fmaf(acc[t][m][j], SPLIT_DOWN, bias_r[t][j]);
             }
         }
+#ifndef INNFER_GRID2_LATE
+        if constexpr (GRID2) {
+            if (c == p.nchunks - 1) {
+                if constexpr (RLDS) { if (p.res2) residual_prefetch_grid2(p, p.res2, p.res2_gstride, rpre, n, ty0, tx0, cwr, li, cbase); }
+                else { if (p.res1) residual_prefetch_grid2(p, p.res1, p.res1_gstride, rpre, n, ty0, tx0, cwr, li, cbase); }
+            }
+        }
+#endif
         const char* st = NSI == 3 ? smem + islot * IN_BYTES : smem + (g & 1) * STAGE;
         const char* sw = NSI == 3 ? smem + 3 * IN_BYTES + (g & 1) * W_BYTES : st + IN_BYTES;
         if constexpr (NSI == 3) islot = islot == 2 ? 0 : islot + 1;
@@ -612,8 +635,9 @@
         } else if constexpr (TM == TAPS_3X3 && PIPE && !UP4) {
             constexpr int GPS = 2 * (RPW + 2);
             constexpr int NB = 3 * GPS;
+            constexpr int RING = GRID2 ? 4 : 3, AHEAD = RING - 1;
             f16x8 a[3][NT];
-            f16x8 bq[3];
+            f16x8 bq[RING];
             auto lda = [&](int sc, int r) {
 #pragma unroll
                 for (int t = 0; t < NT; ++t) a[r][t] = *(const f16x8*)(sw + aoffs + ((r * 3 + sc) * WROWS + t * 16) * 64);
@@ -623,22 +647,23 @@
                 return *(const f16x8*)(st + boffs[sc][rr & 1] + (rr * LWP + seg * 16) * 64);
             };
             lda(0, 0); lda(0, 1); lda(0, 2);
-            bq[0] = ldb(0); bq[1] = ldb(1);
+#pragma unroll
+            for (int i = 0; i < AHEAD; ++i) bq[i] = ldb(i);
             if constexpr (BRELU) bq[0] = relu_frag(bq[0]);
 #pragma unroll
             for (int i = 0; i < NB; ++i) {
                 const int sc = i / GPS, j = i - sc * GPS, rr = j >> 1, seg = j & 1;
-                if (i + 2 < NB) bq[(i + 2) % 3] = ldb(i + 2);
+                if (i + AHEAD < NB) bq[(i + AHEAD) % RING] = ldb(i + AHEAD);
 #pragma unroll
                 for (int r = 0; r < 3; ++r) {
                     const int rw = rr - r;
                     if (rw >= 0 && rw < RPW) {
 #pragma unroll
                         for (int t = 0; t < NT; ++t)
-                            acc[t][rw * 2 + seg] = __builtin_amdgcn_mfma_f32_16x16x32_f16(a[r][t], bq[i % 3], acc[t][rw * 2 + seg], 0, 0, 0);
+                            acc[t][rw * 2 + seg] = __builtin_amdgcn_mfma_f32_16x16x32_f16(a[r][t], bq[i % RING], acc[t][rw * 2 + seg], 0, 0, 0);
                     }
                 }
-                if constexpr (BRELU) { if (i + 1 < NB) bq[(i + 1) % 3] = relu_frag(bq[(i + 1) % 3]); }
+                if constexpr (BRELU) { if (i + 1 < NB) bq[(i + 1) % RING] = relu_frag(bq[(i + 1) % RING]); }
                 if (sc < 2 && seg == 1) {
                     if (rr == RPW - 1) lda(sc + 1, 0);
                     if (rr == RPW) lda(sc + 1, 1);
@@ -693,7 +718,9 @@
         }
         }
         if constexpr (RLDS) {
-            if constexpr (ROWP) {
+            if constexpr (GRID2) {
+                if (c == p.nchunks - 2 + (cw >> 2)) residual_from_lds_grid2<MT>(acc, st, roffs, p.rs1);
+            } else if constexpr (ROWP) {
                 if (c == p.nchunks - 2) residual_from_lds_plane<MT, 0>(acc, st, roffs, p.rs1);
                 else if (c == p.nchunks - 1) residual_from_lds_plane<MT, 1>(acc, st, roffs, p.rs1);
             } else {
@@ -788,7 +815,7 @@
 
 template <int RPW, int NT, int NLW, int OUTMODE, bool S9, bool POLY, int TM, bool CV, int NSI, int NCW>
 int launch_pc(const KP& kp, int N, hipStream_t s) {
-    constexpr int TH = NCW * RPW;
+    constexpr int TH = PcLayout<RPW, NT, NSI, NCW, TM>::TH;
     constexpr int LDS = PcLayout<RPW, NT, NSI, NCW, TM>::LDS_BYTES;
     static_assert(LDS <= 160 * 1024, "the stages must fit the CU's LDS");
     static_assert(NSI == 2 || (NSI == 3 && !S9 && !POLY), "the three-slot input ring exists for the plain and the canvas loader");
@@ -1062,13 +1089,17 @@
         return launch_pc<2, 4, 4, OUT_SLAB, false, false, TAPS_3X3 | PC_ROWP | PC_PSH>(k, L.N, s);
     }
     if (pc && L.out_mode == OUT_SLAB && nt == 4 && L.stats_part) return launch_pc<2, 4, 4, OUT_SLAB, false, false, TAPS_3X3 | PC_STATS>(k, L.N, s);
+    bool grid2 = pc && L.grid2 && L.out_mode == OUT_SLAB && nt == 4 && L.rowp == 1 && L.K == 64 && L.act <= 2 && INNFER_KNOB("INNFER_GRID2", 1);
+    if (grid2 && INNFER_KNOB("INNFER_CANVAS", 1)) { int gy = 0; long t = 0; grid2 = canvas_grid<16>(k, L.N, &gy, &t) == 0; }
     if (pc && L.out_mode == OUT_SLAB && nt == 4 && L.res1_lds && L.res1 && L.res1 == L.in && L.res1_gstride == L.in_gstride && L.act == 0 && L.K == 64 && L.C >= 96 &&
         !L.up && !L.reflect && L.s1 != 0.f && (L.res1_lds == 2 || L.res2)) {
         k.rs1 = 1.0f / L.s1;
+        if (grid2) return launch_pc<4, 2, 4, OUT_SLAB, false, false, TAPS_3X3 | PC_RLDS | PC_ROWP | PC_GRID2>(k, L.N, s);
         return L.rowp ? launch_pc<2, 4, 4, OUT_SLAB, false, false, TAPS_3X3 | PC_RLDS | PC_ROWP>(k, L.N, s) : launch_pc<2, 4, 4, OUT_SLAB, false, false, TAPS_3X3 | PC_RLDS>(k, L.N, s);
     }
     if (pc && L.out_mode == OUT_SLAB && nt == 4) {
         if (!L.rowp && (INNFER_KNOB("INNFER_FAT", 0) & 2)) return launch_pc<4, 4, 4, OUT_SLAB, false, false, TAPS_3X3, false, 2, 4>(k, L.N, s);
+        if (grid2) return launch_pc<4, 2, 4, OUT_SLAB, false, false, TAPS_3X3 | PC_ROWP | PC_GRID2>(k, L.N, s);
         return L.rowp ? launch_pc<2, 4, 4, OUT_SLAB, false, false, TAPS_3X3 | PC_ROWP>(k, L.N, s) : launch_pc<2, 4, 4>(k, L.N, s);
     }
     if (L.conv7) {
diff --git a/innfer_amd/csrc/conv3x3_epilogue_slab.h b/innfer_amd/csrc/conv3x3_epilogue_slab.h
--- a/innfer_amd/csrc/conv3x3_epilogue_slab.h
+++ b/innfer_amd/csrc/conv3x3_epilogue_slab.h
@@ -118,11 +118,11 @@
     for (int m = 0; m < MT; ++m) {
         ok[m] = PAIR ? (2 * n + (m & 1) < p.N && yw + (m >> 1) < ylim && xl < xlim) : ((yw + (m >> 1) < ylim) && (xl + (m & 1) * 16 < xlim));
         const long o = (m >> 1) * rowstep + (m & 1) * colstep;
-        if (HOIST && R1 && ok[m]) {
+        if (HOIST && R1 && ok[m] ABL_AND(!(p.abl & 512))) {
 #pragma unroll
             for (int t = 0; t < NT; ++t) r1[R1 ? m : 0][t] = *(const f16x4*)(r1b + o + toff_slab<NT, ROWP>(t, p.res1_gstride));
         }
-        if (HOIST && R2 && ok[m]) {
+        if (HOIST && R2 && ok[m] ABL_AND(!(p.abl & 512))) {
 #pragma unroll
             for (int t = 0; t < NT; ++t) r2[R2 ? m : 0][t] = *(const f16x4*)(r2b + o + toff_slab<NT, ROWP>(t, p.res2_gstride));
         }
@@ -178,6 +178,69 @@
     }
 }
 
+struct Grid2Tile { long pix; long rowstep; bool ok[8]; };
+__device__ __forceinline__ Grid2Tile grid2_tile(const KP& p, int n, int ty0, int tx0, int rg, int li, int cbase) {
+    Grid2Tile g;
+    const int yw = ty0 + rg * 4, xl = tx0 + li;
+    g.pix = (((long)n * p.H + yw) * p.W + xl) * 32 + (cbase & 31);
+    g.rowstep = (long)p.W * 32;
+#pragma unroll
+    for (int m = 0; m < 8; ++m) g.ok[m] = (yw + (m >> 1) < p.y1) && (xl + (m & 1) * 16 < p.W);
+    return g;
+}
+__device__ __forceinline__ void residual_prefetch_grid2(const KP& p, const f16* res, long gstride, f16x4 (&rpre)[8][2], int n, int ty0, int tx0, int rg, int li, int cbase) {
+    const int yw = ty0 + rg * 4, xl = tx0 + li;
+    const f16* rb = res + (cbase >> 5) * gstride + (cbase & 31);
+    const int xo[2] = {min(xl, p.W - 1) * 32, min(xl + 16, p.W - 1) * 32};
+#pragma unroll
+    for (int r = 0; r < 4; ++r) {
+        const long ro = ((long)n * p.H + min(yw + r, p.y1 - 1)) * p.W * 32;
+#pragma unroll
+        for (int sg = 0; sg < 2; ++sg)
+#pragma unroll
+            for (int t = 0; t < 2; ++t) rpre[2 * r + sg][t] = *(const f16x4*)(rb + ro + xo[sg] + 4 * t);
+    }
+}
+template <int ACT, bool R1, bool R2, bool SC1, int PRE>
+__device__ __forceinline__ void epilogue_slab_grid2(const KP& p, f32x4 (&acc)[2][8], const f16x4 (&rpre)[8][2], int n, int ty0, int tx0, int rg, int li, int cbase) {
+    static_assert((PRE == 0 && !R1 && !R2) || (PRE == 1 && R1) || (PRE == 2 && R2 && !R1), "the prefetched residual is the one memory residual (res1 when there are two)");
+    const Grid2Tile g = grid2_tile(p, n, ty0, tx0, rg, li, cbase);
+    const int oc0 = cbase + p.out_coff;
+    f16* ob = (f16*)p.out + (oc0 >> 5) * p.out_gstride + (g.pix - (cbase & 31)) + (oc0 & 31);
+    f16x4 r2[(R1 && R2) ? 8 : 1][2];
+    if constexpr (R1 && R2) {
+        const f16* r2b = p.res2 + (cbase >> 5) * p.res2_gstride + g.pix;
+#pragma unroll
+        for (int m = 0; m < 8; ++m) {
+            if (!g.ok[m]) continue;
+#pragma unroll
+            for (int t = 0; t < 2; ++t) r2[m][t] = *(const f16x4*)(r2b + (m >> 1) * g.rowstep + (m & 1) * (16 * 32) + 4 * t);
+        }
+    }
+    __builtin_amdgcn_s_waitcnt(0x0F70);
+#pragma unroll
+    for (int m = 0; m < 8; ++m) {
+        if (!g.ok[m]) continue;
+        f16* op = ob + (m >> 1) * g.rowstep + (m & 1) * (16 * 32);
+#pragma unroll
+        for (int t = 0; t < 2; ++t) {
+            f16x4 h;
+#pragma unroll
+            for (int j = 0; j < 4; ++j) {
+                float f = acc[t][m][j];
+                if (ACT == 1) f = __builtin_amdgcn_fmed3f(f, 0.2f * f, ACT_TOP);
+                else if (ACT == 2) f = __builtin_amdgcn_fmed3f(f, 0.f, ACT_TOP);
+                if (SC1) { f = f * p.s1; FP32_VALUE(f); }
+                if (R1) f = __builtin_fmaf(f, p.s1, (float)rpre[m][t][j]);
+                if (R2) f = __builtin_fmaf(f, p.s2, (float)(PRE == 2 ? rpre[m][t][j] : r2[(R1 && R2) ? m : 0][t][j]));
+                FP32_VALUE(f);
+                h[j] = (f16)f;
+            }
+            *(f16x4*)(op + 4 * t) = h;
+        }
+    }
+}
+
 constexpr float SPLIT_UP = 2048.0f, SPLIT_DOWN = 1.0f / 2048.0f;
 template <int RPW, int NT, int ACT, bool R1, bool R2, bool CV>
 __device__ __forceinline__ void epilogue_slab_split(const KP& p, f32x4 (&acc)[NT][2 * RPW], int n, int ty0, int tx0, int wave, int li, int cbase) {
diff --git a/innfer_amd/csrc/conv3x3_kp.h b/innfer_amd/csrc/conv3x3_kp.h
--- a/innfer_amd/csrc/conv3x3_kp.h
+++ b/innfer_amd/csrc/conv3x3_kp.h
@@ -4,10 +4,12 @@
 
 template <int RPW, int NT, int NSI, int NCW, int TMF>
 struct PcLayout {
-    static constexpr int TH = NCW * RPW;
+    static constexpr bool GRID2 = (TMF & PC_GRID2) != 0;
+    static constexpr int TH = (GRID2 ? NCW / 2 : NCW) * RPW;
+    static constexpr int WROWS = (GRID2 ? 2 : 1) * NT * 16;
     static constexpr int IN_BYTES = (((TH + 2) * LWP + 15) / 16) * 1024;
     static constexpr int NTAP = (TMF & PC_UP4) ? 4 : __builtin_popcount(TMF & TAPS_3X3);
-    static constexpr int W_BYTES = NTAP * NT * 16 * 64;
+    static constexpr int W_BYTES = NTAP * WROWS * 64;
     static constexpr int STAGE = IN_BYTES + W_BYTES;
     static constexpr int TAIL = NSI * IN_BYTES + 2 * W_BYTES;
     static constexpr int FUSE_BYTES = (TMF & PC_FUSE) ? 4096 : 0;
diff --git a/innfer_amd/csrc/conv3x3_modes.h b/innfer_amd/csrc/conv3x3_modes.h
--- a/innfer_amd/csrc/conv3x3_modes.h
+++ b/innfer_amd/csrc/conv3x3_modes.h
@@ -18,6 +18,7 @@
 constexpr int PC_ROWP  = 0x400000;
 constexpr int PC_PSH   = 0x800000;
 constexpr int PC_PRELU = 0x1000000;
+constexpr int PC_GRID2 = 0x2000000;
 
 constexpr int PC_BELOW_FUSE  = PC_FUSE - 1;
 constexpr int PC_BELOW_RLDS  = PC_RLDS - 1;
diff --git a/innfer_amd/csrc/conv3x3_pc_loaders.inc b/innfer_amd/csrc/conv3x3_pc_loaders.inc
--- a/innfer_amd/csrc/conv3x3_pc_loaders.inc
+++ b/innfer_amd/csrc/conv3x3_pc_loaders.inc
@@ -3,7 +3,7 @@
 #ifdef INNFER_PRIO
         __builtin_amdgcn_s_setprio(INNFER_PRIO);
 #else
-        if constexpr (NT <= 2) __builtin_amdgcn_s_setprio(3);
+        if constexpr (NT <= 2 && !GRID2) __builtin_amdgcn_s_setprio(3);
 #endif
 #endif
         const int lw = wave - NCW;
diff --git a/innfer_amd/csrc/conv3x3_pc_tile_end.inc b/innfer_amd/csrc/conv3x3_pc_tile_end.inc
--- a/innfer_amd/csrc/conv3x3_pc_tile_end.inc
+++ b/innfer_amd/csrc/conv3x3_pc_tile_end.inc
@@ -1,4 +1,21 @@
-            if constexpr (OUTMODE == OUT_SLAB && SPLIT) {
+#ifdef INNFER_GRID2_LATE
+            if constexpr (GRID2 && RLDS) { if (p.res2) residual_prefetch_grid2(p, p.res2, p.res2_gstride, rpre, n, ty0, tx0, cwr, li, cbase); }
+            else if constexpr (GRID2) { if (p.res1) residual_prefetch_grid2(p, p.res1, p.res1_gstride, rpre, n, ty0, tx0, cwr, li, cbase); }
+#endif
+            if constexpr (GRID2 && RLDS) {
+                if (p.res2) epilogue_slab_grid2<0, false, true, true, 2>(p, acc, rpre, n, ty0, tx0, cwr, li, cbase);
+                else epilogue_slab_grid2<0, false, false, true, 0>(p, acc, rpre, n, ty0, tx0, cwr, li, cbase);
+            } else if constexpr (GRID2) {
+#define EPI(A, B, C) epilogue_slab_grid2<A, B, C, false, (B) ? 1 : 0>(p, acc, rpre, n, ty0, tx0, cwr, li, cbase)
+            if (!p.res1) {
+                if (p.act == 1) EPI(1, false, false); else if (p.act == 2) EPI(2, false, false); else EPI(0, false, false);
+            } else if (!p.res2) {
+                if (p.act == 1) EPI(1, true, false); else if (p.act == 2) EPI(2, true, false); else EPI(0, true, false);
+            } else {
+                if (p.act == 1) EPI(1, true, true); else if (p.act == 2) EPI(2, true, true); else EPI(0, true, true);
+            }
+#undef EPI
+            } else if constexpr (OUTMODE == OUT_SLAB && SPLIT) {
 #define EPI(A, B, C) epilogue_slab_split<RPW, NT, A, B, C, CV>(p, acc, n, ty0, tx0, cw, li, cbase)
             if (!p.res1) {
                 if (p.act == 1) EPI(1, false, false); else if (p.act == 2) EPI(2, false, false); else EPI(0, false, false);
diff --git a/innfer_amd/csrc/conv3x3_stats_gate_rlds.h b/innfer_amd/csrc/conv3x3_stats_gate_rlds.h
--- a/innfer_amd/csrc/conv3x3_stats_gate_rlds.h
+++ b/innfer_amd/csrc/conv3x3_stats_gate_rlds.h
@@ -128,3 +128,15 @@
             for (int j = 0; j < 4; ++j) acc[2 * HALF + tt][m][j] = __builtin_fmaf((float)x[tt * 4 + j], rs1, acc[2 * HALF + tt][m][j]);
     }
 }
+
+template <int MT>
+__device__ __forceinline__ void residual_from_lds_grid2(f32x4 (&acc)[2][MT], const char* st, const int* roffs, float rs1) {
+#pragma unroll
+    for (int m = 0; m < MT; ++m) {
+        const f16x8 x = *(const f16x8*)(st + roffs[((m >> 1) + 1) & 1] + ((m >> 1) * LWP + (m & 1) * 16) * 64);
+#pragma unroll
+        for (int tt = 0; tt < 2; ++tt)
+#pragma unroll
+            for (int j = 0; j < 4; ++j) acc[tt][m][j] = __builtin_fmaf((float)x[tt * 4 + j], rs1, acc[tt][m][j]);
+    }
+}
diff --git a/innfer_amd/csrc/net.hip b/innfer_amd/csrc/net.hip
--- a/innfer_amd/csrc/net.hip
+++ b/innfer_amd/csrc/net.hip
@@ -128,6 +128,7 @@
 #define INNFER_PS_PC_DEFAULT 1
 #endif
     int ps_pc = INNFER_PS_PC_DEFAULT;
+    int consumer_grid = 1;
     int res_lds = 1;
     bool plus = false;
     int unshuffle = 1;
@@ -465,6 +466,13 @@
     return INNFER_OK;
 }
 
+extern "C" int innfer_net_set_consumer_grid(innfer_net_t net, int mode) {
+    if (!net) return set_error(INNFER_ERR_INVALID, "set_consumer_grid: null network");
+    if (mode < 0 || mode > 1) return set_error(INNFER_ERR_INVALID, "set_consumer_grid: 1 (2 x 4 consumer grid with the residual prefetch: default) or 0 (the 8 x 1 form)");
+    net->consumer_grid = mode;
+    return INNFER_OK;
+}
+
 extern "C" int innfer_net_set_fused_tail(innfer_net_t net, int on) {
     if (!net) return set_error(INNFER_ERR_INVALID, "set_fused_tail: null network");
     net->fused_tail = on ? 1 : 0;
@@ -846,7 +854,9 @@
             if (!c.first && !c.d_w32) return set_error(INNFER_ERR_INVALID, "forward: the fp32-accurate panels of '%s' are missing: call innfer_net_set_precision(net, 1) after the last innfer_net_set_conv", c.key.c_str());
     }
     auto mk = [&](const ConvSlot& cs, const f16* in, long in_g, void* out, long out_g, int N_, int H_, int W_, int act) {
-        return mk_launch(cs, in, in_g, out, out_g, N_, H_, W_, act, LO);
+        ConvLaunch L = mk_launch(cs, in, in_g, out, out_g, N_, H_, W_, act, LO);
+        L.grid2 = net->kind == 0 ? net->consumer_grid : 0;
+        return L;
     };
     f16* fea = (f16*)(ws + cv.fea);
     f16* slab[3] = {(f16*)(ws + cv.slab[0]), (f16*)(ws + cv.slab[1]), (f16*)(ws + cv.slab[2])};
@@ -1206,8 +1216,12 @@
                 : norm::launch_stats((const float*)d_src, cpad, (long)HW, eps, d_gamma, d_beta, d_alpha, d_shift, C, N, d_part, (hipStream_t)stream);
 }
 
-static int conv3x3_f16_impl(const innfer_conv_args* a, const float* d_slope, void* stream);
+static int conv3x3_f16_impl(const innfer_conv_args* a, const float* d_slope, void* stream, int consumer_grid = 1);
 extern "C" int innfer_conv3x3_f16(const innfer_conv_args* a, void* stream) { return conv3x3_f16_impl(a, nullptr, stream); }
+extern "C" int innfer_conv3x3_f16_grid(const innfer_conv_args* a, int consumer_grid, void* stream) {
+    if (consumer_grid < 0 || consumer_grid > 1) return set_error(INNFER_ERR_INVALID, "conv3x3: consumer_grid is 1 (the 2 x 4 consumer grid where the launch has that form) or 0 (the 8 x 1 form)");
+    return conv3x3_f16_impl(a, nullptr, stream, consumer_grid);
+}
 extern "C" int innfer_conv3x3_f16_slope(const innfer_conv_args* a, const float* d_slope, void* stream) { return conv3x3_f16_impl(a, d_slope, stream); }
 
 extern "C" int innfer_shuffle_add(const void* d_slab, int64_t group_stride, const void* d_base, int base_dtype, int normalize, void* d_out, int out_dtype,
@@ -1222,7 +1236,7 @@
     return shuffle_add_launch(T, (hipStream_t)stream);
 }
 
-static int conv3x3_f16_impl(const innfer_conv_args* a, const float* d_slope, void* stream) {
+static int conv3x3_f16_impl(const innfer_conv_args* a, const float* d_slope, void* stream, int consumer_grid) {
     if (!a || !a->d_in || !a->d_packed || !a->d_bias || !a->d_out) return set_error(INNFER_ERR_INVALID, "conv3x3: null argument");
     const bool forms121 = a->conv1x1 || a->prefix_lrelu || a->d_gate_packed || a->d_gate_bias || a->in_relu || a->conv7x7 || a->out_planar || a->out_denorm || a->out_round16 ||
                           a->planar_phases || a->outm;
@@ -1286,6 +1300,7 @@
     L.out_mode = a->pixel_shuffle2 ? OUT_SHUFFLE2 : OUT_SLAB; L.reflect = a->reflect_pad; L.dilation = a->dilation; L.dilation_groups = a->dilation_groups;
     L.res1_lds = a->res1_from_input ? 2 : 0;
     L.slope = d_slope;
+    L.grid2 = consumer_grid;
     L.rowp = a->plane_rows ? 1 : 0;
     if (a->pixel_shuffle2 && a->plane_rows == 2) L.rowp = 2;
     else if (a->pixel_shuffle2 && a->plane_rows) return set_error(INNFER_ERR_INVALID, "conv3x3: pixel_shuffle2 takes plane_rows 0 (innfer_pack_conv3x3 panels) or 2 (innfer_pack_conv3x3_shuffle2 panels)");
diff --git a/innfer_amd/lib.py b/innfer_amd/lib.py
--- a/innfer_amd/lib.py
+++ b/innfer_amd/lib.py
@@ -113,6 +113,7 @@
     "innfer_net_set_fused_tail": (C.c_int, [C.c_void_p, C.c_int]),
     "innfer_net_set_hr_chain": (C.c_int, [C.c_void_p, C.c_int]),
     "innfer_net_set_residual_lds": (C.c_int, [C.c_void_p, C.c_int]),
+    "innfer_net_set_consumer_grid": (C.c_int, [C.c_void_p, C.c_int]),
     "innfer_net_set_upconv_phases": (C.c_int, [C.c_void_p, C.c_int]),
     "innfer_net_set_final_act": (C.c_int, [C.c_void_p, C.c_int]),
     "innfer_net_flops": (C.c_double, [C.c_void_p, C.c_int, C.c_int, C.c_int]),
@@ -178,6 +179,7 @@
     "innfer_pack_convt2x_rows": (C.c_int, [C.c_void_p, C.c_int, C.c_int, C.c_int, C.c_int, C.c_void_p]),
     "innfer_conv3x3_f16": (C.c_int, [C.POINTER(ConvArgs), C.c_void_p]),
     "innfer_conv3x3_f16_slope": (C.c_int, [C.POINTER(ConvArgs), C.c_void_p, C.c_void_p]),
+    "innfer_conv3x3_f16_grid": (C.c_int, [C.POINTER(ConvArgs), C.c_int, C.c_void_p]),
     "innfer_shuffle_add": (C.c_int, [C.c_void_p, C.c_int64, C.c_void_p, C.c_int, C.c_int, C.c_void_p, C.c_int] + [C.c_int] * 5 + [C.c_void_p]),
     "innfer_compact_create": (C.c_int, [C.POINTER(C.c_void_p)] + [C.c_int] * 5),
     "innfer_net_set_conv_slope": (C.c_int, [C.c_void_p, C.c_int, C.c_void_p]),
```

Result: faster. 502.6 MPix/s (median of 6 runs) (+1.6%).
